# chao1224/GeoSSL

Measured on AMD Instinct MI355X. Metric: molecules/s/GPU SchNet+DDM fwd+bwd (QM9-sized, bs=1024); % HBM roofline, higher is better.
Workload: dtype f32

## Files before the change

### geossl_amd/NCSN.py

```python
import ctypes as C
import os

import numpy as np
import torch
from .switches import env as _env
import torch.nn as nn
import torch.nn.functional as F

from . import _lib
from ._lib import call, ptr, stream
from .layout import get_super_edge_layout


class MultiLayerPerceptron(nn.Module):

    def __init__(self, input_dim, hidden_dims, activation="relu", dropout=0):
        super().__init__()
        self.dims = [input_dim] + hidden_dims
        self.activation = getattr(F, activation) if isinstance(activation, str) else None
        self.dropout = nn.Dropout(dropout) if dropout else None
        self.layers = nn.ModuleList()
        for i in range(len(self.dims) - 1):
            self.layers.append(nn.Linear(self.dims[i], self.dims[i + 1]))
        self.reset_parameters()

    def reset_parameters(self):
        for layer in self.layers:
            nn.init.xavier_uniform_(layer.weight)
            nn.init.constant_(layer.bias, 0.0)

    def forward(self, input):
        from .higher_order import _linear_wide
        _lib.require_cuda(input)
        lead = input.shape[:-1]
        x = input.reshape(-1, input.shape[-1])
        for i, layer in enumerate(self.layers):
            x = _linear_wide(x, layer.weight, layer.bias)
            if i < len(self.layers) - 1:
                if self.activation:
                    x = self.activation(x)
                if self.dropout:
                    x = self.dropout(x)
        return x.reshape(*lead, x.shape[-1])


def _head_params(m):
    i, o = m.input_distance_mlp.layers, m.output_mlp.layers
    return [i[0].weight, i[0].bias, i[1].weight, i[1].bias, o[0].weight, o[0].bias, o[1].weight, o[1].bias,
            o[2].weight, o[2].bias]


_FIELDS = ("in_w1", "in_b1", "in_w2", "in_b2", "o1_w", "o1_b", "o2_w", "o2_b", "o3_w", "o3_b")

_SIDE = {"stream": None, "pending": []}


def set_side_stream(stream):
    _SIDE["stream"] = stream


def join_side_stream():
    if _SIDE["pending"]:
        for ev, _keep in _SIDE["pending"]:
            torch.cuda.current_stream().wait_event(ev)
        _SIDE["pending"].clear()


class _NcsnLoss(torch.autograd.Function):
    @staticmethod
    def forward(ctx, h, distance, noise_level, distance_noise, sel, sigmas, anneal_power, out_scale, *params):
        dev = h.device
        S, Fd = sel.S, h.size(1)
        training = ctx.needs_input_grad[0] or any(ctx.needs_input_grad[8:])
        ps = [p.detach().contiguous() for p in params]
        w = _lib.NcsnWeights()
        for name, p in zip(_FIELDS, ps):
            setattr(w, name, ptr(p))
        w.sigmas = ptr(sigmas)
        ctx.grad_slot = getattr(h, "_geossl_grad_slot", None)
        h = h.detach().contiguous()
        loss_e = torch.empty(S, dtype=torch.float32, device=dev)
        sv = None
        saved = {}
        if training:
            saved = dict(a1=torch.empty(S, Fd, dtype=torch.float32, device=dev),
                         a2=torch.empty(S, Fd // 2, dtype=torch.float32, device=dev),
                         pd=torch.empty(S, dtype=torch.float32, device=dev),
                         emb=torch.empty(S, dtype=torch.float32, device=dev),
                         gscale=torch.empty(S, dtype=torch.float32, device=dev))
            sv = _lib.NcsnSaved(*[ptr(saved[k]) for k in ("a1", "a2", "pd", "emb", "gscale")])
        lib = _lib.load()
        nws = max(int(lib.geossl_ddm_loss_fwd_workspace_floats(Fd)), 256)
        ws = (torch.empty if S > 0 else torch.zeros)(nws, dtype=torch.float32, device=dev)
        st = stream()
        call("geossl_ddm_loss_fwd", ptr(h), ptr(sel.batch), ptr(sel.sei0), ptr(sel.sei1), S,
             ptr(distance.contiguous()), ptr(noise_level.contiguous()), ptr(distance_noise.contiguous()), C.byref(w),
             Fd, float(anneal_power), ptr(loss_e), C.byref(sv) if sv is not None else None, ptr(ws), st)
        loss = torch.empty((), dtype=torch.float32, device=dev)
        call("geossl_loss_reduce_partials", ptr(ws), ptr(sel.stats), float(out_scale), ptr(loss), 0, st)
        if training:
            ctx.sel, ctx.ps, ctx.w, ctx.saved, ctx.h = sel, ps, w, saved, h
            ctx.params = params
            ctx.sigmas = sigmas
            ctx.out_scale = float(out_scale)
        return loss

    @staticmethod
    def backward(ctx, gout):
        sel, ps, w, saved, h = ctx.sel, ctx.ps, ctx.w, ctx.saved, ctx.h
        dev = h.device
        S, Fd, N = sel.S, h.size(1), h.size(0)
        st = stream()
        sv = _lib.NcsnSaved(*[ptr(saved[k]) for k in ("a1", "a2", "pd", "emb", "gscale")])
        dfeat = torch.empty(S, Fd, dtype=torch.float32, device=dev)
        demb = torch.empty(S, dtype=torch.float32, device=dev)
        grow = torch.empty(S, dtype=torch.float32, device=dev)
        gout = gout.contiguous().to(torch.float32)
        direct = _lib.direct_grads_enabled(ctx.params)
        grads = [p.grad for p in ctx.params] if direct else [torch.empty_like(p) for p in ps]
        g = _lib.NcsnGrads(*[ptr(t) for t in grads])
        lib = _lib.load()
        acc = 1 if direct else 0
        split = (_env("GEOSSL_NCSN_SPLIT_BWD") is not None or _env("GEOSSL_ARITH_24BIT") is not None
                 or max(S, N) * Fd * 4 >= 2 ** 32)
        if not split:
            ws1 = torch.empty(int(lib.geossl_ddm_loss_bwd_fused_workspace_floats(S, Fd)), dtype=torch.float32, device=dev)
            call("geossl_ddm_loss_bwd_fused", ptr(h), ptr(sel.sei0), ptr(sel.sei1), S, N, Fd, C.byref(w), C.byref(sv),
                 ptr(sel.stats), ctx.out_scale, ptr(gout), ptr(dfeat), ptr(demb), ptr(grow), C.byref(g), ptr(ws1), acc, st)
            dz1 = None
        else:
            dz1 = torch.empty(S, Fd, dtype=torch.float32, device=dev)
            call("geossl_ddm_loss_bwd_rows", C.byref(w), C.byref(sv), S, Fd, ptr(sel.stats), ctx.out_scale, ptr(gout),
                 ptr(dz1), ptr(dfeat), ptr(demb), ptr(grow), st)
        dh = None
        if ctx.needs_input_grad[0]:
            slot = ctx.grad_slot
            dh = slot.rows(N, Fd, torch.float32, dev) if slot is not None else None
            if dh is None:
                dh = torch.empty(N, Fd, dtype=torch.float32, device=dev)
            call("geossl_incidence_gather", ptr(dfeat), ptr(sel.inc_ptr), ptr(sel.inc_idx), N, Fd, ptr(dh), 0, st)
        if split:
            nfl = lib.geossl_ddm_loss_bwd_workspace_floats(S, Fd)
            side = _SIDE["stream"] if direct else None
            if side is None:
                ws = torch.empty(nfl, dtype=torch.float32, device=dev)
                call("geossl_ddm_loss_bwd_weights", ptr(h), ptr(sel.sei0), ptr(sel.sei1), S, Fd, C.byref(w), C.byref(sv),
                     ptr(dz1), ptr(demb), ptr(grow), C.byref(g), ptr(ws), acc, st)
            else:
                main = torch.cuda.current_stream()
                fork = torch.cuda.Event()
                fork.record(main)
                side.wait_event(fork)
                with torch.cuda.stream(side):
                    ws = torch.empty(nfl, dtype=torch.float32, device=dev)
                    call("geossl_ddm_loss_bwd_weights", ptr(h), ptr(sel.sei0), ptr(sel.sei1), S, Fd, C.byref(w),
                         C.byref(sv), ptr(dz1), ptr(demb), ptr(grow), C.byref(g), ptr(ws), 1, stream())
                    done = torch.cuda.Event()
                    done.record(side)
                _SIDE["pending"].append((done, (h, saved, dz1, demb, grow, ws, w, sv, ps, grads)))
        if direct:
            return (dh, None, None, None, None, None, None, None) + (None,) * len(grads)
        return (dh, None, None, None, None, None, None, None) + tuple(grads)


class _NcsnLossPair(torch.autograd.Function):

    @staticmethod
    def forward(ctx, h1, h2, d1, d2, nl1, dn1, nl2, dn2, sel, sigmas, powers, out_scale, npar, *params):
        dev = h1.device
        S, Fd, N = sel.S, h1.size(1), h1.size(0)
        training = ctx.needs_input_grad[0] or ctx.needs_input_grad[1] or any(ctx.needs_input_grad[13:])
        ps = [p.detach().contiguous() for p in params]
        pss = (ps[:npar], ps[npar:])
        dyn = getattr(sel, "dyn", None)
        ctx.dyn = dyn
        if dyn is not None:
            hs = (h1.detach().contiguous(),) * 2
            ctx.grad_slots = (None, None)
        else:
            hs = (h1.detach().contiguous(), h2.detach().contiguous())
            ctx.grad_slots = (getattr(h1, "_geossl_grad_slot", None), getattr(h2, "_geossl_grad_slot", None))
        heads = (_lib.NcsnHeadFwd * 2)()
        keep, saved, ws = [], [], []
        for k, (h, d, nl, dn) in enumerate(((hs[0], d1, nl1, dn1), (hs[1], d2, nl2, dn2))):
            hd = heads[k]
            d, nl, dn = d.contiguous(), nl.contiguous(), dn.contiguous()
            keep += [d, nl, dn]
            for name, p in zip(_FIELDS, pss[k]):
                setattr(hd.w, name, ptr(p))
            hd.w.sigmas = ptr(sigmas[k])
            hd.h, hd.distance, hd.noise_level, hd.distance_noise = ptr(h), ptr(d), ptr(nl), ptr(dn)
            hd.anneal_power = float(powers[k])
            loss_e = torch.empty(S, dtype=torch.float32, device=dev)
            sv = {}
            if training:
                sv = dict(a1=torch.empty(S, Fd, dtype=torch.float32, device=dev),
                          a2=torch.empty(S, Fd // 2, dtype=torch.float32, device=dev),
                          pd=torch.empty(S, dtype=torch.float32, device=dev),
                          emb=torch.empty(S, dtype=torch.float32, device=dev),
                          gscale=torch.empty(S, dtype=torch.float32, device=dev))
                for name in ("a1", "a2", "pd", "emb", "gscale"):
                    setattr(hd.saved, name, ptr(sv[name]))
            w_ = torch.empty(256, dtype=torch.float32, device=dev)
            hd.loss_e, hd.workspace = ptr(loss_e), ptr(w_)
            keep.append(loss_e)
            saved.append(sv)
            ws.append(w_)
        st = stream()
        call("geossl_ddm_loss_fwd2_dyn", C.byref(heads), ptr(sel.batch), ptr(sel.sei0), ptr(sel.sei1), S, Fd,
             None if dyn is None else dyn.n_super, None if dyn is None else dyn.n_atoms, st)
        loss = torch.empty((), dtype=torch.float32, device=dev)
        call("geossl_loss_reduce_partials2", ptr(ws[0]), ptr(ws[1]), ptr(sel.stats), float(out_scale), float(out_scale),
             ptr(loss), st)
        if training:
            ctx.sel, ctx.pss, ctx.saved, ctx.hs, ctx.sigmas = sel, pss, saved, hs, sigmas
            ctx.params, ctx.npar, ctx.out_scale = params, npar, float(out_scale)
        return loss

    @staticmethod
    def backward(ctx, gout):
        sel, pss, saved, hs = ctx.sel, ctx.pss, ctx.saved, ctx.hs
        dev = hs[0].device
        S, Fd, N = sel.S, hs[0].size(1), hs[0].size(0)
        st = stream()
        gout = gout.contiguous().to(torch.float32)
        direct = _lib.direct_grads_enabled(ctx.params)
        grads = [p.grad for p in ctx.params] if direct else [torch.empty_like(p) for p in pss[0] + pss[1]]
        gs = (grads[:ctx.npar], grads[ctx.npar:])
        lib = _lib.load()
        heads = (_lib.NcsnHeadBwd * 2)()
        keep, dhs = [], []
        nws = int(lib.geossl_ddm_loss_bwd_fused_workspace_floats(S, Fd))
        dyn = ctx.dyn
        dh_all = torch.empty(N, Fd, dtype=torch.float32, device=dev) if dyn is not None else None
        for k in range(2):
            hd = heads[k]
            for name, p in zip(_FIELDS, pss[k]):
                setattr(hd.w, name, ptr(p))
            hd.w.sigmas = ptr(ctx.sigmas[k])
            for name in ("a1", "a2", "pd", "emb", "gscale"):
                setattr(hd.saved, name, ptr(saved[k][name]))
            for name, t_ in zip(_FIELDS, gs[k]):
                setattr(hd.grads, name, ptr(t_))
            dfeat = torch.empty(S, Fd, dtype=torch.float32, device=dev)
            demb = torch.empty(S, dtype=torch.float32, device=dev)
            grow = torch.empty(S, dtype=torch.float32, device=dev)
            ws1 = torch.empty(nws, dtype=torch.float32, device=dev)
            slot = ctx.grad_slots[k]
            dh = dh_all if dyn is not None else (slot.rows(N, Fd, torch.float32, dev) if slot is not None else None)
            if dh is None:
                dh = torch.empty(N, Fd, dtype=torch.float32, device=dev)
            hd.h, hd.out_scale, hd.dfeat, hd.demb, hd.grow, hd.workspace, hd.dh = (
                ptr(hs[k]), ctx.out_scale, ptr(dfeat), ptr(demb), ptr(grow), ptr(ws1), ptr(dh))
            keep += [dfeat, demb, grow, ws1]
            dhs.append(dh)
        call("geossl_ddm_loss_bwd_fused2_dyn", C.byref(heads), ptr(sel.sei0), ptr(sel.sei1), S, sel.N if dyn is not None else N,
             Fd, ptr(sel.stats), ptr(gout), ptr(sel.inc_ptr), ptr(sel.inc_idx), 1 if direct else 0,
             None if dyn is None else dyn.n_super, None if dyn is None else dyn.n_atoms, st)
        head = ((dh_all, None) if dyn is not None else (dhs[0], dhs[1])) + (None,) * 11
        if direct:
            return head + (None,) * len(grads)
        return head + tuple(grads)


def ddm_heads_loss(n1, n2, data, h1, distance_1, h2, distance_2, noise_level_1=None, distance_noise_1=None,
                   noise_level_2=None, distance_noise_2=None, out_scale=0.5):
    ok = (isinstance(n1, NCSN_version_03) and isinstance(n2, NCSN_version_03) and n1.emb_dim == n2.emb_dim
          and n1.emb_dim in (32, 64, 128) and not _env("GEOSSL_NCSN_SPLIT_BWD")
          and not _env("GEOSSL_ARITH_24BIT")
          and not _env("GEOSSL_NCSN_SEPARATE_HEADS")
          and (h2 is None or h1.shape == h2.shape) and not distance_1.requires_grad and not distance_2.requires_grad
          and n1 is not n2 and not ({id(p) for p in _head_params(n1)} & {id(p) for p in _head_params(n2)}))
    if ok:
        S_, N_, Fd = data.super_edge_index.size(1), h1.size(0), h1.size(1)
        ok = S_ > 0 and max(S_, N_) * Fd * 4 < 2 ** 32
    bucket = getattr(data, "_bucket", None)
    if bucket is not None and (not ok or h2 is not None):
        raise _lib.GeosslHipError("a capacity-bucket batch needs the paired NCSN heads on one fused feature tensor")
    if not ok:
        return (n1(data, h1, distance_1, noise_level=noise_level_1, distance_noise=distance_noise_1, out_scale=out_scale) +
                n2(data, h2, distance_2, noise_level=noise_level_2, distance_noise=distance_noise_2, out_scale=out_scale))
    _lib.require_cuda(h1, h2, distance_1, distance_2, n1.sigmas, n2.sigmas)
    n1.device = n2.device = n1.sigmas.device
    num_graphs = data.num_graphs
    sel = bucket.sel if bucket is not None else get_super_edge_layout(data.batch, data.super_edge_index, num_graphs)
    draws = []
    for n_, nl, dn, d in ((n1, noise_level_1, distance_noise_1, distance_1), (n2, noise_level_2, distance_noise_2, distance_2)):
        if nl is None:
            nl = torch.randint(0, n_.sigmas.size(0), (num_graphs,), device=n_.sigmas.device)
        if dn is None:
            dn = torch.randn_like(d)
        draws.append((nl, dn))
    p1, p2 = _head_params(n1), _head_params(n2)
    return _NcsnLossPair.apply(h1, h2, distance_1.view(-1), distance_2.view(-1), draws[0][0], draws[0][1].view(-1),
                               draws[1][0], draws[1][1].view(-1), sel, (n1.sigmas.detach(), n2.sigmas.detach()),
                               (n1.anneal_power, n2.anneal_power), out_scale, len(p1), *p1, *p2)


class NCSN_version_03(torch.nn.Module):
    def __init__(self, emb_dim, sigma_begin, sigma_end, num_noise_level, noise_type, anneal_power):
        super().__init__()
        self.anneal_power = anneal_power
        self.noise_type = noise_type
        self.input_distance_mlp = MultiLayerPerceptron(1, [emb_dim, 1], activation="relu")
        self.output_mlp = MultiLayerPerceptron(1 + emb_dim, [emb_dim, emb_dim // 2, 1])
        sigmas = torch.tensor(np.exp(np.linspace(np.log(sigma_begin), np.log(sigma_end), num_noise_level)),
                              dtype=torch.float32)
        self.sigmas = nn.Parameter(sigmas, requires_grad=False)
        self.emb_dim = emb_dim

    def forward(self, data, node_feature, distance, debug=False, noise_level=None, distance_noise=None,
                out_scale=1.0):
        self.device = self.sigmas.device
        _lib.require_cuda(node_feature, distance, self.sigmas)
        if self.emb_dim not in (32, 64, 128):
            raise NotImplementedError("HIP path supports emb_dim in (32, 64, 128)")
        if distance.requires_grad:
            raise NotImplementedError("gradient w.r.t. distance/positions is not built (SURVEY.md §8(f) N3)")
        num_graphs = data.num_graphs
        sel = get_super_edge_layout(data.batch, data.super_edge_index, num_graphs)
        if noise_level is None:
            noise_level = torch.randint(0, self.sigmas.size(0), (num_graphs,), device=self.device)
        if distance_noise is None:
            distance_noise = torch.randn_like(distance)
        if sel.S == 0:
            raise ValueError("batch has no super edges (scatter_add over an empty index fails in the reference too)")
        loss = _NcsnLoss.apply(node_feature, distance.view(-1), noise_level, distance_noise.view(-1), sel,
                               self.sigmas.detach(), self.anneal_power, out_scale, *_head_params(self))
        if debug:
            print("loss", float(loss))
        return loss
```

### geossl_amd/_lib.py

```python
import ctypes as C
import os

import torch

HERE = os.path.dirname(os.path.abspath(__file__))
LIB_PATH = os.path.join(HERE, "lib", "libgeossl_hip.so")

MAX_L = 12
TN_MAX = 32
EPI_BIAS, EPI_SSP, EPI_RESIDUAL, EPI_MUL_DSSP, CHAIN_SAME_INPUT, CHAIN_NEW_INPUT, CHAIN_ADD_PREV = 1, 2, 4, 8, 16, 32, 64
EPI_SILU, EPI_MUL_DSILU = 128, 256

vp = C.c_void_p
i64 = C.c_int64
i32 = C.c_int
f32 = C.c_float
f64 = C.c_double
u64 = C.c_uint64


class FilterWeights(C.Structure):
    _fields_ = [("w1", vp * MAX_L), ("b1", vp * MAX_L), ("w2", vp * MAX_L), ("b2", vp * MAX_L)]


PREPARE_MAX = 64


class PrepareBatch(C.Structure):
    _fields_ = [("W", vp * PREPARE_MAX), ("image", vp * PREPARE_MAX), ("ldw", i32 * PREPARE_MAX), ("tb", i32 * PREPARE_MAX)]


CHAIN_MAX = 5


class ChainStage(C.Structure):
    _fields_ = [("image", vp), ("bias", vp), ("res", vp), ("tprev", vp), ("out", vp), ("ld", i32), ("flags", i32),
                ("xin", vp), ("ldxin", i32), ("pad_", i32), ("out_act", vp)]


class Chain(C.Structure):
    _fields_ = [("nstage", i32), ("st", ChainStage * CHAIN_MAX)]


LOOP_MAX_OPS = 14


class LoopOp(C.Structure):
    _fields_ = [("kind", i32), ("swap", i32), ("X", vp), ("Wf", vp), ("out", vp), ("chain", Chain)]


class FilterGradIn(C.Structure):
    _fields_ = [("x", vp * MAX_L), ("dagg", vp * MAX_L)]


class FilterGradOut(C.Structure):
    _fields_ = [("dw1", vp * MAX_L), ("db1", vp * MAX_L), ("dw2", vp * MAX_L), ("db2", vp * MAX_L)]


class TnBatch(C.Structure):
    _fields_ = [("A", vp * TN_MAX), ("B", vp * TN_MAX), ("dW", vp * TN_MAX), ("db", vp * TN_MAX)]


class NcsnWeights(C.Structure):
    _fields_ = [(k, vp) for k in ("in_w1", "in_b1", "in_w2", "in_b2", "o1_w", "o1_b", "o2_w", "o2_b", "o3_w", "o3_b",
                                  "sigmas")]


class NcsnGrads(C.Structure):
    _fields_ = [(k, vp) for k in ("in_w1", "in_b1", "in_w2", "in_b2", "o1_w", "o1_b", "o2_w", "o2_b", "o3_w", "o3_b")]


class NcsnSaved(C.Structure):
    _fields_ = [(k, vp) for k in ("a1", "a2", "pd", "emb", "gscale")]


class NcsnHeadFwd(C.Structure):
    _fields_ = [("h", vp), ("distance", vp), ("noise_level", vp), ("distance_noise", vp), ("w", NcsnWeights),
                ("saved", NcsnSaved), ("anneal_power", f32), ("pad_", f32), ("loss_e", vp), ("workspace", vp)]


class NcsnHeadBwd(C.Structure):
    _fields_ = [("h", vp), ("w", NcsnWeights), ("saved", NcsnSaved), ("out_scale", f32), ("pad_", f32), ("dfeat", vp),
                ("demb", vp), ("grow", vp), ("grads", NcsnGrads), ("workspace", vp), ("dh", vp)]


COPY_MAX = 8


class CopyBatch(C.Structure):
    _fields_ = [("dst", vp * COPY_MAX), ("src", vp * COPY_MAX), ("bytes", i64 * COPY_MAX)]


class Gather(C.Structure):
    _fields_ = [(k, vp) for k in ("x_src", "pos_src", "src_off", "mol_ptr", "x_dst", "pos_dst", "batch_dst", "se_ptr", "sei0",
                                  "sei1", "pair_ptr2", "pair_i", "pair_j", "inc_ptr", "inc_idx", "e0_src", "e1_src",
                                  "e_src_off", "e_ptr", "e0_dst", "e1_dst", "zero")] + \
               [("zero_count", i64), ("x_cols", i32), ("option", i32)]


class Mask(C.Structure):
    _fields_ = [(k, vp) for k in ("bond_ptr", "bond_dst", "src_n", "mol_id", "keep_in", "keep_out", "e_src_cnt",
                                  "e_count")] + [("seed", u64), ("max_n", i32), ("pad_", i32)]


P = C.POINTER
PROTOTYPES = {
    "geossl_abi_version": (i32, []),
    "geossl_layout_build": (i32, [vp, i64, i64, vp, vp, vp, vp]),
    "geossl_pair_index_fill": (i32, [vp, vp, i64, vp, vp, vp]),
    "geossl_radius_graph_count": (i32, [vp, vp, i64, i32, f32, i32, vp, vp]),
    "geossl_radius_graph_fill": (i32, [vp, vp, i64, i32, f32, i32, vp, vp, vp, vp, vp]),
    "geossl_pair_geometry": (i32, [vp, vp, vp, i64, i32, f32, i32, f32, vp, vp, vp, vp]),
    "geossl_rbf_fwd": (i32, [vp, i64, vp, i32, f32, vp, vp]),
    "geossl_ssp_fwd": (i32, [vp, i64, vp, vp]),
    "geossl_ssp_bwd": (i32, [vp, vp, i64, vp, vp]),
    "geossl_cfconv_filter_fwd": (i32, [vp, vp, i64, P(FilterWeights), i32, i32, i32, vp, f32, vp, vp, vp]),
    "geossl_cfconv_filter_bwd_workspace_floats": (i64, [i64, i32, i32, i32]),
    "geossl_cfconv_filter_bwd": (i32, [vp, vp, vp, vp, vp, i64, i64, P(FilterWeights), P(FilterGradIn), i32, i32, i32, vp,
                                       f32, vp, P(FilterGradOut), vp, i32, vp]),
    "geossl_cfconv_filter_dpos": (i32, [vp, vp, vp, vp, vp, i64, P(FilterWeights), P(FilterGradIn), i32, i32, i32, vp, f32,
                                        f32, vp, vp, vp, vp]),
    "geossl_pair_position_grad": (i32, [vp, vp, vp, vp, vp, i64, i64, i32, vp, vp]),
    "geossl_cfconv_aggregate": (i32, [vp, vp, vp, vp, vp, vp, i64, i32, i32, i32, vp, vp]),
    "geossl_aggregate_parts": (i32, [i32]),
    "geossl_cfconv_aggregate_work": (i32, [vp, vp, vp, vp, vp, vp, i64, i32, i32, i32, vp, vp]),
    "geossl_pair_product": (i32, [vp, vp, vp, vp, vp, i64, i32, i32, vp, vp]),
    "geossl_linear": (i32, [vp, i32, vp, vp, vp, vp, vp, i32, i64, i32, i32, i32, i32, vp]),
    "geossl_tn_plan": (None, [i64, i32, P(i32), P(i32)]),
    "geossl_tn_workspace_floats": (i64, [i64, i32, i32, i32]),
    "geossl_row_normalize_fwd": (i32, [vp, i64, i32, f32, vp, vp, vp]),
    "geossl_row_normalize_bwd": (i32, [vp, vp, vp, i64, i32, f32, vp, vp]),
    "geossl_atom_tuples": (i32, [vp, vp, i64, i32, vp, vp, vp]),
    "geossl_linear_image_words": (i64, [i32, i32]),
    "geossl_linear_prepare": (i32, [P(PrepareBatch), i32, i32, i32, i32, vp]),
    "geossl_linear_prepared": (i32, [vp, i32, vp, vp, vp, vp, vp, i32, i64, i32, i32, i32, vp]),
    "geossl_chain_image_words": (i64, [i32]),
    "geossl_chain_prepare": (i32, [P(PrepareBatch), i32, i32, i32, vp]),
    "geossl_linear_chain": (i32, [vp, i32, P(Chain), i64, i32, vp]),
    "geossl_linear_wgrad": (i32, [P(TnBatch), i32, i64, i32, i32, i32, i32, i32, vp, i32, vp]),
    "geossl_embedding_fwd": (i32, [vp, i64, vp, i32, i64, i32, vp, vp, vp]),
    "geossl_embedding_bwd_workspace_floats": (i64, [i32, i32]),
    "geossl_embedding_bwd": (i32, [vp, i64, vp, i32, i64, i32, vp, vp, i32, vp]),
    "geossl_segment_reduce_fwd": (i32, [vp, vp, i64, i32, i32, vp, vp]),
    "geossl_segment_reduce_bwd": (i32, [vp, vp, i64, i32, i32, vp, i32, vp]),
    "geossl_axpy": (i32, [vp, vp, f32, i64, vp, vp]),
    "geossl_pair_distance": (i32, [vp, vp, vp, i64, vp, vp]),
    "geossl_super_edge_ptr": (i32, [vp, vp, vp, i64, i64, vp, vp, vp]),
    "geossl_incidence_count": (i32, [vp, vp, vp, vp, i64, i32, vp, vp]),
    "geossl_incidence_fill": (i32, [vp, vp, vp, vp, i64, i32, vp, vp, vp]),
    "geossl_ddm_loss_fwd_workspace_floats": (i64, [i32]),
    "geossl_ddm_loss_fwd": (i32, [vp, vp, vp, vp, i64, vp, vp, vp, P(NcsnWeights), i32, f32, vp, P(NcsnSaved), vp, vp]),
    "geossl_schnet_layer_loop": (i32, [vp, i32, vp, i32, vp, vp, vp, i32, i32, i64, i32, i32, vp]),
    "geossl_schnet_layer_loop_ragged": (i32, [vp, i32, vp, vp, vp, i64, i32, i64, i32, vp]),
    "geossl_copy2": (i32, [vp, vp, i64, vp, vp, i64, vp]),
    "geossl_ddm_noise": (i32, [vp, f32, f32, i64, i64, i64, i32, i32, vp, vp, vp, vp, vp, vp]),
    "geossl_ddm_noise_seeded": (i32, [u64, f32, f32, i64, i64, i64, i32, i32, vp, vp, vp, vp, vp, vp]),
    "geossl_ddm_views": (i32, [vp, vp, vp, vp, i64, i64, vp, vp, vp, vp, i64, vp, vp]),
    "geossl_loss_reduce_partials": (i32, [vp, vp, f32, vp, i32, vp]),
    "geossl_ddm_loss_fwd2": (i32, [vp, vp, vp, vp, i64, i32, vp]),
    "geossl_loss_reduce_partials2": (i32, [vp, vp, vp, f32, f32, vp, vp]),
    "geossl_ddm_loss_bwd_fused2": (i32, [vp, vp, vp, i64, i64, i32, vp, vp, vp, vp, i32, vp]),
    "geossl_loss_reduce_workspace_floats": (i64, [i64]),
    "geossl_loss_reduce": (i32, [vp, i64, vp, f32, vp, vp, i32, vp]),
    "geossl_ddm_loss_bwd_rows": (i32, [P(NcsnWeights), P(NcsnSaved), i64, i32, vp, f32, vp, vp, vp, vp, vp, vp]),
    "geossl_ddm_loss_bwd_workspace_floats": (i64, [i64, i32]),
    "geossl_ddm_loss_bwd_weights": (i32, [vp, vp, vp, i64, i32, P(NcsnWeights), P(NcsnSaved), vp, vp, vp, P(NcsnGrads),
                                          vp, i32, vp]),
    "geossl_ddm_loss_bwd_fused_workspace_floats": (i64, [i64, i32]),
    "geossl_ddm_loss_bwd_fused": (i32, [vp, vp, vp, i64, i64, i32, P(NcsnWeights), P(NcsnSaved), vp, f32, vp, vp, vp, vp,
                                        P(NcsnGrads), vp, i32, vp]),
    "geossl_incidence_gather": (i32, [vp, vp, vp, i64, i32, vp, i32, vp]),
    "geossl_painn_edge_geom": (i32, [vp, vp, vp, i64, f32, vp, vp, i32, vp, vp, vp, vp]),
    "geossl_silu_fwd": (i32, [vp, i64, vp, vp]),
    "geossl_silu_bwd": (i32, [vp, vp, i64, vp, vp]),
    "geossl_painn_interaction_fwd": (i32, [vp, vp, vp, vp, vp, vp, vp, vp, vp, vp, vp, i64, i32, i32, vp, vp, vp]),
    "geossl_painn_interaction_bwd_workspace_floats": (i64, [i64, i32, i32]),
    "geossl_painn_interaction_fwd_mol": (i32, [vp, vp, vp, vp, vp, vp, vp, vp, vp, vp, vp, vp, i64, i32, i64, i32, i32, vp,
                                               vp, vp]),
    "geossl_painn_interaction_fwd_mma": (i32, [vp, vp, vp, vp, vp, vp, vp, vp, vp, vp, vp, vp, vp, i64, i32, i64, i32, i32,
                                               vp, vp, vp]),
    "geossl_painn_interaction_bwd_mol_workspace_floats": (i64, [i64, i64, i32, i32]),
    "geossl_painn_interaction_bwd_mol": (i32, [vp, vp, vp, vp, vp, vp, vp, vp, vp, vp, vp, vp, vp, i64, i32, i64, i32, i32,
                                               vp, vp, vp, vp, vp, i32, vp]),
    "geossl_painn_interaction_bwd": (i32, [vp, vp, vp, vp, vp, vp, vp, vp, vp, vp, vp, vp, i64, i32, i32, vp, vp, vp, vp,
                                           vp, i32, vp]),
    "geossl_painn_mix_pre_fwd": (i32, [vp, vp, i64, i32, f32, vp, vp, vp]),
    "geossl_painn_mix_post_fwd": (i32, [vp, vp, vp, vp, vp, i64, i32, vp, vp, vp]),
    "geossl_painn_mix_post_bwd": (i32, [vp, vp, vp, vp, vp, i64, i32, vp, vp, vp]),
    "geossl_painn_mix_pre_bwd": (i32, [vp, vp, vp, vp, i64, i32, vp, vp, vp]),
    "geossl_add": (i32, [vp, vp, i64, vp, vp]),
    "geossl_painn_edge_grads": (i32, [vp] * 11 + [i64, i32, i32, vp, vp, vp, i32, vp]),
    "geossl_painn_edge_geom_bwd": (i32, [vp, vp, vp, i64, f32, vp, vp, i32, vp, vp, vp, vp, vp]),
    "geossl_painn_position_grad": (i32, [vp, vp, vp, vp, vp, i64, vp, vp]),
    "geossl_adam_step": (i32, [vp, vp, vp, vp, i64, f64, f64, f64, f64, f64, i64, f32, vp]),
    "geossl_copy_n": (i32, [P(CopyBatch), i32, vp]),
    "geossl_ddm_views_dyn": (i32, [vp, vp, vp, vp, i64, i64, vp, vp, vp, vp, i64, vp, vp, vp, vp]),
    "geossl_embedding_fwd_dyn": (i32, [vp, i64, vp, i32, i64, i32, vp, vp, vp, vp]),
    "geossl_embedding_bwd_dyn": (i32, [vp, i64, vp, i32, i64, i32, vp, vp, i32, vp, vp]),
    "geossl_cfconv_filter_fwd_dyn": (i32, [vp, vp, i64, P(FilterWeights), i32, i32, i32, vp, f32, vp, vp, vp, vp]),
    "geossl_cfconv_filter_bwd_dyn": (i32, [vp, vp, vp, vp, vp, i64, i64, P(FilterWeights), P(FilterGradIn), i32, i32, i32,
                                           vp, f32, vp, P(FilterGradOut), vp, i32, vp, vp, vp]),
    "geossl_rbf_fragments_bytes": (i64, [i64]),
    "geossl_rbf_fragments": (i32, [vp, i64, i32, vp, f32, vp, vp]),
    "geossl_rbf_fragments_dyn": (i32, [vp, i64, i32, vp, f32, vp, vp, vp]),
    "geossl_rbf_fragment_items": (i32, [vp, i64, i32, vp, f32, vp, vp, vp]),
    "geossl_cfconv_filter_bwd_frag": (i32, [vp, vp, vp, vp, vp, i64, i64, P(FilterWeights), P(FilterGradIn), i32, i32,
                                            i32, vp, f32, vp, P(FilterGradOut), vp, i32, vp, vp]),
    "geossl_cfconv_filter_bwd_frag_dyn": (i32, [vp, vp, vp, vp, vp, i64, i64, P(FilterWeights), P(FilterGradIn), i32,
                                                i32, i32, vp, f32, vp, P(FilterGradOut), vp, i32, vp, vp, vp, vp]),
    "geossl_cfconv_aggregate_work_dyn": (i32, [vp, vp, vp, vp, vp, vp, i64, i32, i32, i32, vp, vp, vp]),
    "geossl_cfconv_aggregate_targets_dyn": (i32, [vp, vp, vp, vp, vp, vp, i64, i32, i32, i32, vp, vp, vp]),
    "geossl_linear_chain_dyn": (i32, [vp, i32, P(Chain), i64, i32, vp, vp]),
    "geossl_linear_wgrad_dyn": (i32, [P(TnBatch), i32, i64, i32, i32, i32, i32, i32, vp, i32, vp, vp]),
    "geossl_ddm_loss_fwd2_dyn": (i32, [vp, vp, vp, vp, i64, i32, vp, vp, vp]),
    "geossl_ddm_loss_bwd_fused2_dyn": (i32, [vp, vp, vp, i64, i64, i32, vp, vp, vp, vp, i32, vp, vp, vp]),
    "geossl_painn_group_capacity": (i64, [i64, i64]),
    "geossl_painn_edge_layout": (i32, [vp, vp, i64, vp, i64, i64, i64] + [vp] * 12),
    "geossl_painn_edge_layout_dyn": (i32, [vp, vp, i64, vp, vp, i64, i64, i64] + [vp] * 12),
    "geossl_painn_edge_geom_dyn": (i32, [vp, vp, vp, i64, f32, vp, vp, i32, vp, vp, vp, vp, vp]),
    "geossl_painn_interaction_fwd_mma_dyn": (i32, [vp, vp, vp, vp, vp, vp, vp, vp, vp, vp, vp, vp, vp, i64, i32, i64, i32,
                                                   i32, vp, vp, vp, vp]),
    "geossl_tape_unary": (i32, [i32, vp, i64, f32, f32, vp, vp]),
    "geossl_tape_binary": (i32, [i32, vp, i32, vp, i32, i64, i32, f32, vp, vp]),
    "geossl_tape_colsum_workspace_floats": (i64, [i64, i32]),
    "geossl_tape_reduce": (i32, [i32, vp, i64, i32, vp, vp, vp]),
    "geossl_tape_gather_rows": (i32, [vp, vp, i32, i64, i32, vp, vp]),
    "geossl_tape_scatter_rows": (i32, [vp, vp, i32, vp, i64, i32, vp, vp]),
    "geossl_tape_copy2d": (i32, [vp, i64, vp, i64, i64, i32, vp]),
    "geossl_tape_fill": (i32, [vp, i64, f32, vp]),
    "geossl_painn_stage_cap": (i32, [i32, i32, i32]),
    "geossl_painn_interaction_fwd_atoms": (i32, [vp] * 12 + [i64, vp, i32, i32, vp, vp, vp]),
    "geossl_painn_interaction_bwd_atoms": (i32, [vp] * 13 + [i64, vp, i32, i32, vp, vp, vp, vp, vp, i32, vp]),
    "geossl_painn_tile_ok": (i32, [i32, i32]),
    "geossl_painn_interaction_fwd_tile": (i32, [vp] * 12 + [i64, vp, i32, i32, vp, vp, vp]),
    "geossl_painn_interaction_bwd_tile_workspace_floats": (i64, [i64, i32, i32]),
    "geossl_painn_interaction_bwd_tile": (i32, [vp] * 13 + [i64, vp, i32, i32, vp, vp, vp, vp, vp, i32, vp]),
    "geossl_painn_interaction_bwd_mol_skip": (i32, [vp, vp, vp, vp, vp, vp, vp, vp, vp, vp, vp, vp, vp, i64, i32, i64, i32,
                                                    i32, vp, vp, vp, vp, vp, i32, vp]),
    "geossl_painn_mix_pre_fwd_dyn": (i32, [vp, vp, i64, i32, f32, vp, vp, vp, vp]),
    "geossl_painn_mix_post_fwd_dyn": (i32, [vp, vp, vp, vp, vp, i64, i32, vp, vp, vp, vp]),
    "geossl_painn_mix_post_bwd_dyn": (i32, [vp, vp, vp, vp, vp, i64, i32, vp, vp, vp, vp]),
    "geossl_painn_mix_pre_bwd_dyn": (i32, [vp, vp, vp, vp, i64, i32, vp, vp, vp, vp]),
    "geossl_gather_molecules": (i32, [P(Gather), i64, vp]),
    "geossl_gather_masked_molecules": (i32, [P(Gather), P(Mask), i64, vp]),
    "geossl_masked_edge_offsets": (i32, [vp, i64, i64, i32, vp, vp, vp, vp]),
    "geossl_infonce_fwd": (i32, [vp, vp, i64, i32, f32, vp, vp, vp, vp, vp]),
    "geossl_infonce_bwd": (i32, [vp, vp, vp, vp, i64, i32, f32, vp, vp, vp, vp]),
    "geossl_ebm_nce_fwd": (i32, [vp, vp, i64, i32, i32, vp, vp, vp, vp, vp, vp]),
    "geossl_ebm_nce_bwd": (i32, [vp, vp, vp, i64, i32, i32, vp, vp, vp, vp]),
    "geossl_distance_head_width_ok": (i32, [i32]),
    "geossl_distance_head_fwd_workspace_floats": (i64, [i64]),
    "geossl_distance_head_bwd_workspace_floats": (i64, [i64, i32]),
    "geossl_distance_head_fwd": (i32, [vp, i64, i32, vp, vp, vp, vp, vp, i64, vp, vp, vp, vp, vp, vp]),
    "geossl_distance_head_fwd_dyn": (i32, [vp, i64, i32, vp, vp, vp, vp, vp, i64, vp, vp, vp, vp, vp, vp, vp, vp]),
    "geossl_distance_head_bwd": (i32, [vp, i64, i32, vp, vp, i64, vp, vp, vp, vp, vp, vp, vp, vp, i32, vp]),
    "geossl_distance_head_bwd_dyn": (i32, [vp, i64, i32, vp, vp, i64, vp, vp, vp, vp, vp, vp, vp, vp, i32, vp, vp, vp]),
    "geossl_charge_mask_count": (i64, [i64, f64]),
    "geossl_charge_mask": (i32, [vp, i32, i64, f64, i32, vp, vp, vp, vp, vp, vp]),
    "geossl_charge_mask_dyn": (i32, [vp, i32, i64, f64, i32, vp, vp, vp, vp, vp, vp, vp]),
    "geossl_charge_head_width_ok": (i32, [i32, i32]),
    "geossl_charge_head_fwd_workspace_floats": (i64, [i64]),
    "geossl_charge_head_bwd_workspace_floats": (i64, [i64, i32, i32]),
    "geossl_charge_head_fwd": (i32, [vp, i64, i32, vp, vp, i32, vp, vp, i64, vp, vp, vp, vp, vp, vp]),
    "geossl_charge_head_fwd_dyn": (i32, [vp, i64, i32, vp, vp, i32, vp, vp, i64, vp, vp, vp, vp, vp, vp, vp]),
    "geossl_charge_head_bwd": (i32, [vp, i64, i32, vp, i32, vp, vp, i64, vp, vp, vp, vp, vp, vp, vp, i32, vp]),
    "geossl_charge_head_bwd_dyn": (i32, [vp, i64, i32, vp, i32, vp, vp, i64, vp, vp, vp, vp, vp, vp, vp, i32, vp, vp]),
    "geossl_infograph_width_ok": (i32, [i32]),
    "geossl_infograph_fwd_workspace_floats": (i64, [i64]),
    "geossl_infograph_fwd": (i32, [vp, i64, i32, vp, vp, i64, i32, vp, vp, vp, vp, vp, vp, vp, vp]),
    "geossl_infograph_fwd_dyn": (i32, [vp, i64, i32, vp, vp, i64, i32, vp, vp, vp, vp, vp, vp, vp, vp, vp]),
    "geossl_infograph_bwd": (i32, [vp, i64, i32, vp, vp, i64, i32, vp, vp, vp, vp, vp, vp, vp, vp]),
    "geossl_infograph_bwd_dyn": (i32, [vp, i64, i32, vp, vp, i64, i32, vp, vp, vp, vp, vp, vp, vp, vp, vp]),
    "geossl_property_width_ok": (i32, [i32]),
    "geossl_property_workspace_floats": (i64, [i64]),
    "geossl_property_fwd": (i32, [vp, i64, i32, vp, i64, i32, i32, vp, vp, vp, vp, vp, i64, vp, i32, vp, vp, vp, vp, vp,
                                  vp]),
    "geossl_property_fwd_dyn": (i32, [vp, i64, i32, vp, i64, i32, i32, vp, vp, vp, vp, vp, i64, vp, i32, vp, vp, vp, vp,
                                      vp, vp, vp]),
    "geossl_property_predict": (i32, [vp, i64, i32, vp, i64, i32, i32, vp, vp, vp, vp, vp, vp, vp]),
    "geossl_property_predict_dyn": (i32, [vp, i64, i32, vp, i64, i32, i32, vp, vp, vp, vp, vp, vp, vp, vp]),
    "geossl_property_bwd": (i32, [i64, i32, vp, i64, i32, i32, vp, vp, vp, vp, vp, vp, i64, vp, i32, vp, vp, vp, vp, vp,
                                  vp, i32, vp]),
    "geossl_property_bwd_dyn": (i32, [i64, i32, vp, i64, i32, i32, vp, vp, vp, vp, vp, vp, i64, vp, i32, vp, vp, vp, vp,
                                      vp, vp, i32, vp, vp]),
    "geossl_property_targets": (i32, [vp, i64, i32, i32, vp, vp, i64, vp, vp]),
    "geossl_pair_head_width_ok": (i32, [i32]),
    "geossl_pair_head_workspace_floats": (i64, [i64]),
    "geossl_pair_head_fwd": (i32, [vp, i64, i32, vp, i64, i32, vp, vp, vp, vp, vp, vp, vp, vp]),
    "geossl_pair_head_predict": (i32, [vp, i64, i32, vp, i64, i32, vp, vp, vp, vp]),
    "geossl_pair_head_bwd": (i32, [i64, i32, vp, i64, i32, vp, vp, vp, vp, vp, vp, vp, vp, vp, i32, vp]),
    "geossl_pair_head_fwd_dyn": (i32, [vp, i64, i32, vp, i64, i32, vp, vp, vp, vp, vp, vp, vp, vp, vp]),
    "geossl_pair_head_predict_dyn": (i32, [vp, i64, i32, vp, i64, i32, vp, vp, vp, vp, vp]),
    "geossl_pair_head_bwd_dyn": (i32, [i64, i32, vp, i64, i32, vp, vp, vp, vp, vp, vp, vp, vp, vp, i32, vp, vp]),
    "geossl_torsion_head_width_ok": (i32, [i32]),
    "geossl_torsion_head_fwd_workspace_floats": (i64, [i64]),
    "geossl_torsion_head_bwd_workspace_floats": (i64, [i64, i32]),
    "geossl_torsion_head_fwd": (i32, [vp, i64, i32, vp, vp, vp, vp, vp, vp, i64, vp, vp, vp, vp, vp, vp]),
    "geossl_torsion_head_fwd_dyn": (i32, [vp, i64, i32, vp, vp, vp, vp, vp, vp, i64, vp, vp, vp, vp, vp, vp, vp, vp]),
    "geossl_torsion_head_bwd": (i32, [vp, i64, i32, vp, vp, vp, vp, i64, vp, vp, i64, vp, vp, vp, vp, vp, i32, vp]),
    "geossl_torsion_head_bwd_dyn": (i32, [vp, i64, i32, vp, vp, vp, vp, i64, vp, vp, i64, vp, vp, vp, vp, vp, i32, vp, vp,
                                          vp]),
    "geossl_triple_angles": (i32, [vp, i64, vp, vp, vp, i64, vp, vp]),
    "geossl_gather_triples": (i32, [vp, i64, vp, vp, vp, vp, i64, vp, vp, vp, vp, vp]),
    "geossl_sparse_pairs_build": (i32, [vp, vp, i64, i64, i32, f32, i32, f32, i64] + [vp] * 13),
    "geossl_cfconv_aggregate_sparse": (i32, [vp, vp, vp, vp, vp, i64, i32, i32, vp, vp]),
    "geossl_sparse_pairs_build_dyn": (i32, [vp, vp, i64, i64, i32, f32, i32, f32, i64] + [vp] * 14),
    "geossl_cfconv_aggregate_sparse_dyn": (i32, [vp, vp, vp, vp, vp, i64, i32, i32, vp, vp, vp]),
    "geossl_pair_position_grad_sparse": (i32, [vp, vp, vp, vp, vp, vp, i64, i64, i32, vp, vp]),
    "geossl_pair_geometry_live": (i32, [vp, vp, vp, i64, i32, f32, i32, f32, vp, vp, vp, vp, vp]),
    "geossl_gather_live_rows": (i32, [vp, vp, vp, i64, i32, i32, vp, vp]),
    "geossl_live_pairs_build": (i32, [vp] * 8 + [i64, i64, f32] + [vp] * 9),
    "geossl_cfconv_filter_fwd_rows": (i32, [vp, vp, i64, P(FilterWeights), i32, i32, i32, vp, f32, vp, vp, vp, vp, vp]),
}

_lib = None


class GeosslHipError(RuntimeError):
    pass


def load():
    global _lib
    if _lib is not None:
        return _lib
    path = os.environ.get("GEOSSL_HIP_LIB", LIB_PATH)
    if not os.path.exists(path):
        raise GeosslHipError(
            "libgeossl_hip.so is not built (%s). Run `python -m geossl_amd.build` (needs hipcc); "
            "there is no CPU fallback." % path)
    lib = C.CDLL(path)
    for name, (res, args) in PROTOTYPES.items():
        fn = getattr(lib, name)
        fn.restype = res
        fn.argtypes = args
    if lib.geossl_abi_version() != 1:
        raise GeosslHipError("ABI version mismatch")
    _lib = lib
    return lib


def check(rc, what):
    if rc != 0:
        raise GeosslHipError("%s failed with hipError %d" % (what, rc))


def ptr(t):
    if t is None:
        return None
    return t.data_ptr()


def stream():
    return torch._C._cuda_getCurrentRawStream(torch._C._cuda_getDevice())


def require_cuda(*tensors):
    for t in tensors:
        if t is not None and not t.is_cuda:
            raise GeosslHipError(
                "geossl_amd runs on MI355X only: got a %s tensor. The HIP path has no CPU fallback." % t.device.type)



_DIRECT = {"depth": 0}


class direct_grads:
    def __enter__(self):
        _DIRECT["depth"] += 1
        return self

    def __exit__(self, *exc):
        _DIRECT["depth"] -= 1
        return False


def direct_grads_enabled(params):
    return _DIRECT["depth"] > 0 and all(
        p.grad is not None and p.grad.is_contiguous() and p.grad.dtype == torch.float32 and p.grad.is_cuda
        for p in params)


class StatusWord:

    def __init__(self, device, message):
        self.word = torch.zeros(1, dtype=torch.int32, device=device)
        self.host = torch.zeros(1, dtype=torch.int32).pin_memory()
        self.event = None
        self.message = message

    def __deepcopy__(self, memo):
        return None

    def __reduce__(self):
        return (type(None), ())

    def poll(self):
        if self.event is None or torch.cuda.is_current_stream_capturing():
            return
        if self.event.query():
            self.event = None
            if int(self.host[0]):
                raise IndexError(self.message)

    def arm(self, every=1):
        self.calls = getattr(self, "calls", 0) + 1
        if every > 1 and self.calls % every != 1:
            return
        if self.event is None and not torch.cuda.is_current_stream_capturing():
            self.host.copy_(self.word, non_blocking=True)
            self.event = torch.cuda.Event()
            self.event.record()

    def check(self):
        if int(self.word.item()):
            raise IndexError(self.message)


def module_status(module, device, message):
    st = module.__dict__.get("_geossl_status")
    if st is None or st.word.device != device:
        st = StatusWord(device, message)
        module.__dict__["_geossl_status"] = st
    return st


TIMERS = None
CALLS = None


def call(name, *args):
    global CALLS
    lib = load()
    if CALLS is not None:
        CALLS += 1
    timers = TIMERS
    key = name[:-4] if name.endswith("_dyn") else name
    if key == "geossl_cfconv_filter_fwd_rows":
        key = "geossl_cfconv_filter_fwd"
    if timers is not None and key in timers:
        e0, e1 = torch.cuda.Event(enable_timing=True), torch.cuda.Event(enable_timing=True)
        e0.record()
        rc = getattr(lib, name)(*args)
        e1.record()
        timers[key].append((e0, e1))
    else:
        rc = getattr(lib, name)(*args)
    check(rc, name)


def fill_ptrs(arr, tensors):
    for i, t in enumerate(tensors):
        arr[i] = ptr(t)
```

### geossl_amd/csrc/ncsn_bwd.hip

```cpp
#include "common.h"
#include "geossl_hip.h"
#include "split.h"
#include "tn.h"

using namespace geossl;

namespace {

constexpr int TR = 32;

#ifdef NB_TIMING
__device__ long long nb_dbg[2 * 32 * 8];
#define NB_MARK(slot)                                                                              \
  do {                                                                                             \
    if (blockIdx.x == 5 && lane == 0 && (wave == 0 || wave == NW) && t - t_begin < 32)             \
      nb_dbg[((wave == 0 ? 0 : 1) * 32 + (t - t_begin)) * 8 + (slot)] = clock64();                 \
  } while (0)
#else
#define NB_MARK(slot) do {} while (0)
#endif

template <int NW>
struct NbLds {
  static constexpr int F = 32 * NW, H = F / 2, KHS = (H + 15) / 16, HMB = (H + 31) / 32, KS = F / 16;
  u32x4* zb;
  u32x4* dz2T;
  u32x4* fT;
  u32x4* dz1r;
  u32x4* abT;
  int4* scal;
  float* pdv;
  float* dep;
  float* wls;
  int* eg;
  int* ef;
  int* ea;
  int* ec;
  __device__ explicit NbLds(uint8_t* smem) {
    zb = reinterpret_cast<u32x4*>(smem);
    dz2T = zb + 2 * KHS * 2 * 64;
    fT = dz2T + HMB * 2 * 2 * 64;
    dz1r = fT + 2 * NW * 2 * 2 * 64;
    abT = dz1r + KS * 2 * 64;
    scal = reinterpret_cast<int4*>(abT + NW * 2 * 2 * 64);
    pdv = reinterpret_cast<float*>(scal + 3 * TR);
    dep = pdv + 3 * TR;
    wls = dep + NW * TR;
    eg = reinterpret_cast<int*>(wls + F);
    ef = eg + 4;
    ea = ef + 2 * NW;
    ec = ea + NW;
  }
  static size_t bytes() {
    return (size_t)(2 * KHS * 2 + HMB * 4 + 2 * NW * 4 + KS * 2 + NW * 4) * 1024 + 3 * TR * sizeof(int4) +
           (size_t)(3 * TR + NW * TR + F) * sizeof(float) + (size_t)(4 + 4 * NW) * sizeof(int);
  }
};

struct NcsnFusedArgs {
  const float* h;
  const int64_t* sei0;
  const int64_t* sei1;
  int S;
  GeosslNcsnWeights w;
  GeosslNcsnSaved sv;
  const int64_t* divisor;
  float out_scale;
  const float* gout;
  float* dfeat;
  float* demb;
  float* grow;
  float* pw1;
  float* pd1;
  float* pb1;
  float* pw2;
  float* pb2;
  float* psm;
};

__device__ __forceinline__ float ldg_off(const float* base, uint32_t byte_off) {
  return *reinterpret_cast<const float*>(reinterpret_cast<const char*>(base) + byte_off);
}
__device__ __forceinline__ int crow4(int r, int k4) { return (r & 3) + 8 * (r >> 2) + k4; }
__device__ __forceinline__ int opaque(int v) {
  asm volatile("" : "+v"(v));
  return v;
}
__device__ __forceinline__ u32x4 pack8(const f32x16& t, int s) {
  u32x4 w;
#pragma unroll
  for (int q = 0; q < 4; ++q) {
    const f16x2 p = {(_Float16)t[8 * s + 2 * q], (_Float16)t[8 * s + 2 * q + 1]};
    w[q] = __builtin_bit_cast(uint32_t, p);
  }
  return w;
}
__device__ __forceinline__ const u32x4& piece(const Frag2& f, int pc) { return pc == 0 ? f.h : f.l; }
__device__ __forceinline__ int scale_exponent(float m) { return max(mag_exponent(m), -40); }
__device__ __forceinline__ float pow2(int e) { return __builtin_amdgcn_ldexpf(1.0f, e); }
constexpr int E_NONE = -100000;

template <int NW, bool ROLE_A>
__device__ __forceinline__ void ncsn_bwd_body(const NcsnFusedArgs& a, const int S, const float* __restrict__ a_h) {
  using L_t = NbLds<NW>;
  constexpr int F = L_t::F, H = L_t::H, KHS = L_t::KHS, HMB = L_t::HMB, KS = L_t::KS, NT = 128 * NW;
  extern __shared__ __attribute__((aligned(16))) uint8_t smem_raw[];
  const L_t L(smem_raw);
  const int tid = threadIdx.x, lane = tid & 63, j = lane & 31, kh = lane >> 5;
  const int wave = __builtin_amdgcn_readfirstlane(tid >> 6);
  const int nb = ROLE_A ? wave : wave - NW;
  const int ntiles = (S + TR - 1) / TR;
  const int per = (ntiles + (int)gridDim.x - 1) / (int)gridDim.x;
  const int t_begin = (int)blockIdx.x * per, t_end = min(ntiles, t_begin + per);
  const float scale = a.out_scale * (a.gout != nullptr ? a.gout[0] : 1.0f) / (float)a.divisor[0];
  const uint32_t col = 32 * nb + j;

  Frag2 wreg[ROLE_A ? KHS : KS];
  f32x16 accw1[ROLE_A ? NW : 1];
  f32x16 accw2[ROLE_A ? 1 : HMB];
  int E1[ROLE_A ? NW : 1];
  int E2 = E_NONE;
  int ew = 0;
  float bsum = 0.0f, dsum = 0.0f;
  u32x4 ident[2];
  float w3r[8];
  float s_w2 = 0.0f, s_w1 = 0.0f, s_b1 = 0.0f, s_g = 0.0f, s_d = 0.0f;
  float iw1 = 0.0f, ib1 = 0.0f, iw2 = 0.0f;
  int e3;
  {
    float m3 = 0.0f;
    for (int i = lane; i < H; i += 64) m3 = fmaxf(m3, fabsf(a.w.o3_w[i]));
    e3 = scale_exponent(wave_max(m3));
  }
  if constexpr (ROLE_A) {
    iw1 = a.w.in_w1[col];
    ib1 = a.w.in_b1[col];
    iw2 = a.w.in_w2[col];
    float raw[KHS][8];
    float wm = 0.0f, csum = 0.0f;
#pragma unroll
    for (int ks = 0; ks < KHS; ++ks)
#pragma unroll
      for (int e = 0; e < 8; ++e) {
        const int m = 16 * ks + 8 * kh + e;
        const float v = m < H ? a.w.o2_w[(size_t)m * F + col] : 0.0f;
        raw[ks][e] = v;
        wm = fmaxf(wm, fabsf(v));
        csum = fmaf(fabsf(v), m < H ? fabsf(a.w.o3_w[m]) : 0.0f, csum);
      }
    ew = scale_exponent(wave_max(wm));
    const float sw = pow2(14 - ew);
#pragma unroll
    for (int ks = 0; ks < KHS; ++ks) wreg[ks] = split8h_scaled(raw[ks], sw);
    csum += __shfl_xor(csum, 32, 64);
    const int ecw = max(mag_exponent(wave_max(csum)), -80);
    if (lane == 0) L.ec[nb] = ecw;
#pragma unroll
    for (int kb = 0; kb < NW; ++kb) {
      E1[kb] = E_NONE;
#pragma unroll
      for (int r = 0; r < 16; ++r) accw1[kb][r] = 0.0f;
    }
#pragma unroll
    for (int s = 0; s < 2; ++s)
#pragma unroll
      for (int q = 0; q < 4; ++q) {
        const int k0 = 16 * s + kperm(2 * q, kh), k1 = 16 * s + kperm(2 * q + 1, kh);
        ident[s][q] = (k0 == j ? 0x3C00u : 0u) | (k1 == j ? 0x3C000000u : 0u);
      }
  } else {
    float raw[KS][8];
    float wm = 0.0f;
#pragma unroll
    for (int ks = 0; ks < KS; ++ks)
#pragma unroll
      for (int e = 0; e < 8; ++e) {
        raw[ks][e] = a.w.o1_w[(size_t)(16 * ks + kperm(e, kh)) * (F + 1) + col];
        wm = fmaxf(wm, fabsf(raw[ks][e]));
      }
    ew = scale_exponent(wave_max(wm));
    const float sw = pow2(14 - ew);
#pragma unroll
    for (int ks = 0; ks < KS; ++ks) wreg[ks] = split8h_scaled(raw[ks], sw);
#pragma unroll
    for (int e = 0; e < 8; ++e) {
      const int m = 16 * nb + 8 * kh + e;
      w3r[e] = (nb < KHS && m < H) ? a.w.o3_w[m] : 0.0f;
    }
#pragma unroll
    for (int mb = 0; mb < HMB; ++mb)
#pragma unroll
      for (int r = 0; r < 16; ++r) accw2[mb][r] = 0.0f;
#pragma unroll
    for (int q2 = 0; q2 < 2; ++q2)
#pragma unroll
      for (int q = 0; q < 4; ++q) {
        const int k0 = 16 * q2 + 8 * kh + 2 * q;
        ident[q2][q] = (k0 == j ? 0x3C00u : 0u) | (k0 + 1 == j ? 0x3C000000u : 0u);
      }
  }
  for (int i = tid; i < F; i += NT) L.wls[i] = a.w.o1_w[(size_t)i * (F + 1) + F];

  int sc_u = 0, sc_v = 0;
  float sc_g = 0.0f, sc_e = 0.0f, sc_p = 0.0f;
  int EG = -60;
  auto load_scal = [&](int tt) {
    if constexpr (ROLE_A) {
      if (wave == 0) {
        const int row = min(TR * tt + j, S - 1);
        sc_u = (int)a.sei0[row];
        sc_v = (int)a.sei1[row];
        sc_g = a.sv.gscale[row];
        sc_e = a.sv.emb[row];
        sc_p = a.sv.pd[row];
      }
    }
  };
  auto put_scal = [&](int tt) {
    if constexpr (ROLE_A) {
      if (wave == 0) {
        const int row = TR * tt + lane;
        const bool valid = lane < TR && row < S && tt < t_end;
        const float gr = valid ? pin(sc_g) * scale : 0.0f;
        EG = max(EG, mag_exponent(wave_max(fabsf(gr))));
        if (lane < TR) {
          L.scal[(tt % 3) * TR + lane] = make_int4(sc_u, sc_v, __float_as_int(gr), __float_as_int(sc_e));
          L.pdv[(tt % 3) * TR + lane] = sc_p;
          if (valid) a.grow[row] = gr;
        }
        if (lane == 0) L.eg[tt % 3] = EG;
      }
    }
  };
  float a1raw[16];
  auto request_a1 = [&](int tt, int k4) {
    if constexpr (ROLE_A) {
#pragma unroll
      for (int r = 0; r < 16; ++r)
        a1raw[r] = ldg_off(a.sv.a1, ((uint32_t)min(TR * tt + crow4(r, k4), S - 1) * (uint32_t)F + col) * 4u);
    }
  };
  f32x4 a2raw[2];
  float o3acc[8] = {0.0f, 0.0f, 0.0f, 0.0f, 0.0f, 0.0f, 0.0f, 0.0f};
  auto request_a2 = [&](int tt) {
    if constexpr (!ROLE_A) {
      if (nb < KHS) {
        const uint32_t off = ((uint32_t)min(TR * tt + j, S - 1) * (uint32_t)H + (16 * nb + 8 * kh)) * 4u;
        a2raw[0] = *reinterpret_cast<const f32x4*>(reinterpret_cast<const char*>(a.sv.a2) + off);
        a2raw[1] = *reinterpret_cast<const f32x4*>(reinterpret_cast<const char*>(a.sv.a2) + 16 + off);
      }
    }
  };
  float hu[16], hv[16];
  auto request_gather = [&](int tt, int k4) {
    if constexpr (!ROLE_A) {
      const int2* sc = reinterpret_cast<const int2*>(L.scal + (tt % 3) * TR);
#pragma unroll
      for (int r = 0; r < 16; ++r) {
        const int2 uv = sc[2 * crow4(r, k4)];
        hu[r] = ldg_off(a_h, ((uint32_t)uv.x * (uint32_t)F + col) * 4u);
        hv[r] = ldg_off(a_h, ((uint32_t)uv.y * (uint32_t)F + col) * 4u);
      }
    }
  };
  auto build_zb = [&](int tt) {
    if constexpr (!ROLE_A) {
      if (nb < KHS) {
        const float gr = __int_as_float(L.scal[(tt % 3) * TR + j].z);
        const float sz = pow2(14 - e3 - __builtin_amdgcn_readfirstlane(L.eg[tt % 3]));
        const float av[8] = {a2raw[0].x, a2raw[0].y, a2raw[0].z, a2raw[0].w, a2raw[1].x, a2raw[1].y, a2raw[1].z, a2raw[1].w};
        float v[8];
#pragma unroll
        for (int e = 0; e < 8; ++e) {
          const float a2v = pin(av[e]);
          v[e] = a2v > 0.0f ? gr * w3r[e] : 0.0f;
          o3acc[e] = fmaf(gr, a2v, o3acc[e]);
        }
        const Frag2 f = split8h_scaled(v, sz);
        u32x4* dst = L.zb + (size_t)(((tt & 1) * KHS + nb) * 2) * 64 + lane;
        dst[0] = f.h;
        dst[64] = f.l;
      }
    }
  };
  int EF = -40;
  auto build_fT = [&](int tt) {
    if constexpr (!ROLE_A) {
      float v[16];
      float m = 0.0f;
#pragma unroll
      for (int r = 0; r < 16; ++r) {
        v[r] = pin(hu[r]) + pin(hv[r]);
        m = fmaxf(m, fabsf(v[r]));
      }
      EF = max(EF, mag_exponent(wave_max(m)));
      const float sf = pow2(14 - EF);
      if (lane == 0) L.ef[(tt & 1) * NW + nb] = EF;
#pragma unroll
      for (int s = 0; s < 2; ++s) {
        float vv[8];
#pragma unroll
        for (int e = 0; e < 8; ++e) vv[e] = v[8 * s + e];
        const Frag2 f = split8h_scaled(vv, sf);
        u32x4* dst = L.fT + (size_t)((((tt & 1) * NW + nb) * 2 + s) * 2) * 64 + lane;
        dst[0] = f.h;
        dst[64] = f.l;
      }
    }
  };

  load_scal(t_begin);
  put_scal(t_begin);
  load_scal(t_begin + 1);
  put_scal(t_begin + 1);
  load_scal(t_begin + 2);
  if (t_begin < t_end) {
    request_a1(t_begin, 4 * kh);
    request_a2(t_begin);
  }
  __syncthreads();
  int eC = -80;
#pragma unroll
  for (int i = 0; i < NW; ++i) eC = max(eC, __builtin_amdgcn_readfirstlane(L.ec[i]));
  if (t_begin < t_end) {
    request_gather(t_begin, 4 * kh);
    build_zb(t_begin);
    build_fT(t_begin);
    request_a2(t_begin + 1);
    request_gather(t_begin + 1, 4 * kh);
  }
  int EA = -40;
  const float kA = pow2(e3 + ew - eC - 14);
  for (int t = t_begin; t < t_end; ++t) {
    const int buf = t & 1;
    int k4 = opaque(4 * kh);
    NB_MARK(0);
    lds_barrier();
    NB_MARK(1);
    const int EGt = __builtin_amdgcn_readfirstlane(L.eg[t % 3]);
    if constexpr (ROLE_A) {
      put_scal(t + 2);
      const float kT = pow2(EGt + eC - 14);
      f32x16 acc0, acc1;
#pragma unroll
      for (int r = 0; r < 16; ++r) acc0[r] = acc1[r] = 0.0f;
      {
        const u32x4* zs = L.zb + (size_t)(buf * KHS * 2) * 64 + lane;
        Frag2 a0, an;
        a0.h = zs[0]; a0.l = zs[64];
#pragma unroll
        for (int ks = 0; ks < KHS; ++ks) {
          if (ks + 1 < KHS) {
            const u32x4* s0 = zs + (size_t)((ks + 1) * 2) * 64;
            an.h = s0[0]; an.l = s0[64];
          }
          __builtin_amdgcn_sched_barrier(0);
          mma3x2(acc0, acc1, a0, wreg[ks]);
          __builtin_amdgcn_sched_barrier(0);
          if (ks + 1 < KHS) a0 = an;
        }
      }
      NB_MARK(5);
      float v[16];
      {
        const int4* sc = L.scal + (t % 3) * TR;
        float tb = 0.0f, td = 0.0f, am = 0.0f;
#pragma unroll
        for (int r = 0; r < 16; ++r) {
          a1raw[r] = pin(a1raw[r]);
          v[r] = a1raw[r] > 0.0f ? (acc0[r] + acc1[r]) * kA : 0.0f;
          tb += v[r];
          td = fmaf(v[r], __int_as_float(sc[crow4(r, k4)].w), td);
          am = fmaxf(am, fabsf(a1raw[r]));
        }
        bsum = fmaf(tb, kT, bsum);
        dsum = fmaf(td, kT, dsum);
        EA = max(EA, mag_exponent(wave_max(am)));
      }
      {
        const float sa = pow2(14 - EA);
        if (lane == 0) L.ea[nb] = EA;
#pragma unroll
        for (int s = 0; s < 2; ++s) {
          float vv[8];
#pragma unroll
          for (int e = 0; e < 8; ++e) vv[e] = a1raw[8 * s + e];
          const Frag2 f = split8h_scaled(vv, sa);
          u32x4* dst = L.abT + (size_t)((nb * 2 + s) * 2) * 64 + lane;
          dst[0] = f.h;
          dst[64] = f.l;
        }
      }
      Frag2 da[2];
#pragma unroll
      for (int s = 0; s < 2; ++s) {
        float vv[8];
#pragma unroll
        for (int e = 0; e < 8; ++e) vv[e] = v[8 * s + e];
        da[s] = split8h(vv);
      }
      {
        float wl[16];
#pragma unroll
        for (int r = 0; r < 16; ++r) wl[r] = L.wls[32 * nb + crow4(r, k4)];
        float de = 0.0f;
#pragma unroll
        for (int pc = 1; pc >= 0; --pc) {
          f32x16 tp;
#pragma unroll
          for (int r = 0; r < 16; ++r) tp[r] = 0.0f;
          tp = mfma_f16(piece(da[0], pc), ident[0], tp);
          tp = mfma_f16(piece(da[1], pc), ident[1], tp);
#pragma unroll
          for (int r = 0; r < 16; ++r) de = fmaf(tp[r], wl[r], de);
#pragma unroll
          for (int half = 0; half < 2; ++half)
            L.dz1r[(size_t)((2 * nb + half) * 2 + pc) * 64 + lane] = pack8(tp, half);
        }
        de += __shfl_xor(de, 32, 64);
        if (kh == 0) L.dep[j * NW + nb] = de * kT;
      }
      NB_MARK(6);
#pragma unroll
      for (int kb = 0; kb < NW; ++kb) {
        const int En = EGt + __builtin_amdgcn_readfirstlane(L.ef[buf * NW + kb]);
        if (En != E1[kb]) {
          const float f = pow2(max(E1[kb] - En, -200));
#pragma unroll
          for (int r = 0; r < 16; ++r) accw1[kb][r] *= f;
          E1[kb] = En;
        }
#pragma unroll
        for (int s = 0; s < 2; ++s) {
          const u32x4* s0 = L.fT + (size_t)(((buf * NW + kb) * 2 + s) * 2) * 64 + lane;
          Frag2 bf;
          bf.h = s0[0]; bf.l = s0[64];
          mma3(accw1[kb], da[s], bf);
        }
      }
    } else {
      if (nb < HMB) {
        float tb = 0.0f;
#pragma unroll
        for (int pc = 1; pc >= 0; --pc) {
          f32x16 tp;
#pragma unroll
          for (int r = 0; r < 16; ++r) tp[r] = 0.0f;
#pragma unroll
          for (int q = 0; q < 2; ++q) {
            if (2 * nb + q < KHS) {
              const u32x4* s0 = L.zb + (size_t)((buf * KHS + 2 * nb + q) * 2 + pc) * 64 + lane;
              tp = mfma_f16(s0[0], ident[q], tp);
            }
          }
#pragma unroll
          for (int r = 0; r < 16; ++r) tb += tp[r];
#pragma unroll
          for (int s = 0; s < 2; ++s) L.dz2T[(size_t)((nb * 2 + s) * 2 + pc) * 64 + lane] = pack8(tp, s);
        }
        bsum = fmaf(tb, pow2(EGt + e3 - 14), bsum);
      }
      NB_MARK(5);
      build_zb(t + 1);
      NB_MARK(6);
      build_fT(t + 1);
    }
    k4 = opaque(4 * kh);
    NB_MARK(2);
    lds_barrier();
    NB_MARK(3);
    if constexpr (ROLE_A) {
      request_a1(t + 1, k4);
      load_scal(t + 3);
      {
        const int4* sc = L.scal + (t % 3) * TR;
        const float* pdr = L.pdv + (t % 3) * TR;
#pragma unroll
        for (int i = 0; i < 16; ++i) {
          const int rl = 4 * k4 + i;
          float de = 0.0f;
#pragma unroll
          for (int n2 = 0; n2 < NW; ++n2) de += L.dep[rl * NW + n2];
          const float pd = pdr[rl];
          const float pre = fmaf(iw1, pd, ib1);
          s_w2 = fmaf(de, fmaxf(pre, 0.0f), s_w2);
          const float dp = pre > 0.0f ? de * iw2 : 0.0f;
          s_w1 = fmaf(dp, pd, s_w1);
          s_b1 += dp;
          if (wave == 0 && j == i) {
            s_g += __int_as_float(sc[rl].z);
            s_d += de;
          }
        }
      }
    } else {
      request_a2(t + 2);
      request_gather(t + 2, k4);
      NB_MARK(7);
      f32x16 acc0, acc1;
#pragma unroll
      for (int r = 0; r < 16; ++r) acc0[r] = acc1[r] = 0.0f;
      {
        const u32x4* zs = L.dz1r + lane;
        Frag2 b0, bn;
        b0.h = zs[0]; b0.l = zs[64];
#pragma unroll
        for (int ks = 0; ks < KS; ++ks) {
          if (ks + 1 < KS) {
            const u32x4* s0 = zs + (size_t)((ks + 1) * 2) * 64;
            bn.h = s0[0]; bn.l = s0[64];
          }
          __builtin_amdgcn_sched_barrier(0);
          mma3x2(acc0, acc1, wreg[ks], b0);
          __builtin_amdgcn_sched_barrier(0);
          if (ks + 1 < KS) b0 = bn;
        }
      }
      const float kD = pow2(EGt + eC + ew - 28);
      f32x16 outp;
#pragma unroll
      for (int r = 0; r < 16; ++r) outp[r] = (acc0[r] + acc1[r]) * kD;
      const int row = TR * t + j;
      if (row < S) {
        const uint32_t off = ((uint32_t)row * (uint32_t)F + 32 * nb + 4 * kh) * 4u;
#pragma unroll
        for (int q = 0; q < 4; ++q)
          *reinterpret_cast<f32x4*>(reinterpret_cast<char*>(a.dfeat) + 32 * q + off) =
              f32x4{outp[4 * q], outp[4 * q + 1], outp[4 * q + 2], outp[4 * q + 3]};
        if (nb == 0 && kh == 0) {
          float de = 0.0f;
#pragma unroll
          for (int n2 = 0; n2 < NW; ++n2) de += L.dep[j * NW + n2];
          a.demb[row] = de;
        }
      }
      {
        const int En = EGt + __builtin_amdgcn_readfirstlane(L.ea[nb]);
        if (En != E2) {
          const float f = pow2(max(E2 - En, -200));
#pragma unroll
          for (int mb = 0; mb < HMB; ++mb)
#pragma unroll
            for (int r = 0; r < 16; ++r) accw2[mb][r] *= f;
          E2 = En;
        }
      }
#pragma unroll
      for (int s = 0; s < 2; ++s) {
        const u32x4* sb = L.abT + (size_t)((nb * 2 + s) * 2) * 64 + lane;
        Frag2 bf;
        bf.h = sb[0]; bf.l = sb[64];
#pragma unroll
        for (int mb = 0; mb < HMB; ++mb) {
          const u32x4* s0 = L.dz2T + (size_t)((mb * 2 + s) * 2) * 64 + lane;
          Frag2 af;
          af.h = s0[0]; af.l = s0[64];
          mma3(accw2[mb], af, bf);
        }
      }
    }
    NB_MARK(4);
  }
  const size_t pb = blockIdx.x;
  if constexpr (ROLE_A) {
    float* P1 = a.pw1 + pb * F * F;
#pragma unroll
    for (int kb = 0; kb < NW; ++kb) {
      const float f = pow2(max(E1[kb] + eC - 28, -200));
#pragma unroll
      for (int r = 0; r < 16; ++r) P1[(size_t)(32 * nb + c_row(r, lane)) * F + 32 * kb + j] = accw1[kb][r] * f;
    }
    const float sb = bsum + __shfl_xor(bsum, 32, 64), sd = dsum + __shfl_xor(dsum, 32, 64);
    if (kh == 0) {
      a.pb1[pb * F + col] = sb;
      a.pd1[pb * F + col] = sd;
    }
    float* Ps = a.psm + pb * (H + 3 * F + 2);
    const float t_w2 = s_w2 + __shfl_xor(s_w2, 32, 64);
    const float t_w1 = s_w1 + __shfl_xor(s_w1, 32, 64), t_b1 = s_b1 + __shfl_xor(s_b1, 32, 64);
    if (kh == 0) {
      Ps[H + col] = t_w2;
      Ps[H + F + col] = t_w1;
      Ps[H + 2 * F + col] = t_b1;
    }
    if (wave == 0) {
      const float tg = wave_sum(s_g), td = wave_sum(s_d);
      if (lane == 0) {
        Ps[H + 3 * F] = tg;
        Ps[H + 3 * F + 1] = td;
      }
    }
  } else {
    float* P2 = a.pw2 + pb * H * F;
    const float f = pow2(max(E2 + e3 - 28, -200));
#pragma unroll
    for (int mb = 0; mb < HMB; ++mb)
#pragma unroll
      for (int r = 0; r < 16; ++r) {
        const int m = 32 * mb + c_row(r, lane);
        if (m < H) P2[(size_t)m * F + col] = accw2[mb][r] * f;
      }
    const float sb = bsum + __shfl_xor(bsum, 32, 64);
    if (nb < HMB && kh == 0 && (int)col < H) a.pb2[pb * H + col] = sb;
    if (nb < KHS) {
      float* Ps = a.psm + pb * (H + 3 * F + 2);
#pragma unroll
      for (int e = 0; e < 8; ++e) {
        float v = o3acc[e];
#pragma unroll
        for (int o = 16; o > 0; o >>= 1) v += __shfl_xor(v, o, 64);
        const int m = 16 * nb + 8 * kh + e;
        if (j == 0 && m < H) Ps[m] = v;
      }
    }
  }
}

template <int NW>
__global__ __launch_bounds__(128 * NW) void k_ncsn_bwd_fused(NcsnFusedArgs a) {
  if ((int)(threadIdx.x >> 6) < NW) ncsn_bwd_body<NW, true>(a, a.S, a.h);
  else ncsn_bwd_body<NW, false>(a, a.S, a.h);
}
struct NcsnFusedPair { NcsnFusedArgs a[2]; };
template <int NW>
__global__ __launch_bounds__(128 * NW) void k_ncsn_bwd_fused2(NcsnFusedPair pr, const int32_t* __restrict__ dyn_S,
                                                              const int32_t* __restrict__ dyn_view) {
  const NcsnFusedArgs& a = pr.a[blockIdx.y];
  const int S = dyn_count(a.S, dyn_S);
  const float* h = a.h;
  if (dyn_view != nullptr && blockIdx.y == 1) h += (size_t)(*dyn_view) * (32 * NW);
  if ((int)(threadIdx.x >> 6) < NW) ncsn_bwd_body<NW, true>(a, S, h);
  else ncsn_bwd_body<NW, false>(a, S, h);
}

__device__ __forceinline__ void ncsn_reduce_all_block(const ReduceMulti& m, int nblk, int accumulate,
                                                      const float* __restrict__ psm, int F, const GeosslNcsnGrads& g,
                                                      float (*red)[64]) {
  const int mb = m.xoff[m.nseg];
  if ((int)blockIdx.x < mb) {
    reduce_multi_block(m, nblk, accumulate, red, 0);
    return;
  }
  const int H = F / 2, len = H + 3 * F + 2;
  const int i = ((int)blockIdx.x - mb) * 4 + (int)(threadIdx.x >> 6), lane = threadIdx.x & 63;
  if (i >= len) return;
  float s = 0.0f;
  for (int b = lane; b < nblk; b += 64) s += psm[(size_t)b * len + i];
  s = wave_sum(s);
  if (lane == 0) {
    float* dst;
    if (i < H) dst = g.o3_w + i;
    else if (i < H + F) dst = g.in_w2 + (i - H);
    else if (i < H + 2 * F) dst = g.in_w1 + (i - H - F);
    else if (i < H + 3 * F) dst = g.in_b1 + (i - H - 2 * F);
    else if (i == H + 3 * F) dst = g.o3_b;
    else dst = g.in_b2;
    *dst = accumulate ? *dst + s : s;
  }
}
__global__ __launch_bounds__(256) void k_ncsn_reduce_all(ReduceMulti m, int nblk, int accumulate,
                                                         const float* __restrict__ psm, int F, GeosslNcsnGrads g) {
  __shared__ float red[4][64];
  ncsn_reduce_all_block(m, nblk, accumulate, psm, F, g, red);
}
__global__ __launch_bounds__(256) void k_ncsn_reduce_all2(ReduceMulti m0, ReduceMulti m1, int nblk, int accumulate,
                                                          const float* __restrict__ psm0,
                                                          const float* __restrict__ psm1, int F, GeosslNcsnGrads g0,
                                                          GeosslNcsnGrads g1) {
  __shared__ float red[4][64];
  if (blockIdx.y == 0) ncsn_reduce_all_block(m0, nblk, accumulate, psm0, F, g0, red);
  else ncsn_reduce_all_block(m1, nblk, accumulate, psm1, F, g1, red);
}

inline int fused_blocks(int64_t S) {
  const int64_t ntiles = (S + TR - 1) / TR;
  return (int)(ntiles < 256 ? ntiles : 256);
}

}

#ifdef NB_TIMING
extern "C" int geossl_ncsn_bwd_debug_read(long long* host) {
  return (int)hipMemcpyFromSymbol(host, HIP_SYMBOL(nb_dbg), sizeof(long long) * 2 * 32 * 8);
}
#endif

extern "C" int64_t geossl_ddm_loss_bwd_fused_workspace_floats(int64_t S, int F) {
  const int64_t nb = fused_blocks(S), H = F / 2;
  return nb * ((int64_t)F * F + 2 * F + H * F + H + (H + 3 * F + 2));
}

extern "C" int geossl_ddm_loss_bwd_fused(const float* h, const int64_t* sei0, const int64_t* sei1, int64_t S, int64_t N,
                                         int F, const GeosslNcsnWeights* w, const GeosslNcsnSaved* saved,
                                         const int64_t* stats_divisor, float out_scale, const float* gout, float* dfeat,
                                         float* demb, float* grow, const GeosslNcsnGrads* grads, float* workspace,
                                         int accumulate, hipStream_t stream) {
  if (S <= 0) return 0;
  if (F != 32 && F != 64 && F != 128) return (int)hipErrorInvalidValue;
  if (S * (int64_t)F * 4 >= ((int64_t)1 << 32) || N * (int64_t)F * 4 >= ((int64_t)1 << 32)) return (int)hipErrorInvalidValue;
  const int nb = fused_blocks(S), H = F / 2;
  NcsnFusedArgs a;
  a.h = h; a.sei0 = sei0; a.sei1 = sei1; a.S = (int)S; a.w = *w; a.sv = *saved; a.divisor = stats_divisor;
  a.out_scale = out_scale; a.gout = gout; a.dfeat = dfeat; a.demb = demb; a.grow = grow;
  a.pw1 = workspace;
  a.pd1 = a.pw1 + (size_t)nb * F * F;
  a.pb1 = a.pd1 + (size_t)nb * F;
  a.pw2 = a.pb1 + (size_t)nb * F;
  a.pb2 = a.pw2 + (size_t)nb * H * F;
  a.psm = a.pb2 + (size_t)nb * H;
#define LAUNCH(NWV)                                                                                      \
  do {                                                                                                   \
    allow_big_lds(&k_ncsn_bwd_fused<NWV>);                                                               \
    hipLaunchKernelGGL((k_ncsn_bwd_fused<NWV>), dim3(nb), dim3(128 * NWV), NbLds<NWV>::bytes(), stream, a); \
  } while (0)
  if (F == 128) LAUNCH(4); else if (F == 64) LAUNCH(2); else LAUNCH(1);
#undef LAUNCH
  GEOSSL_CHECK_LAUNCH();
  ReduceMulti rm;
  float* o1w[1] = {grads->o1_w};
  float* o1c[1] = {grads->o1_w + F};
  float* o1b[1] = {grads->o1_b};
  float* o2w[1] = {grads->o2_w};
  float* o2b[1] = {grads->o2_b};
  rm.add(a.pw1, F * F, F, F + 1, 1, o1w, 1);
  rm.add(a.pd1, F, F, F, F + 1, o1c, 1);
  rm.add(a.pb1, F, F, F, 1, o1b, 1);
  rm.add(a.pw2, H * F, F, F, 1, o2w, 1);
  rm.add(a.pb2, H, H, H, 1, o2b, 1);
  hipLaunchKernelGGL(k_ncsn_reduce_all, dim3(rm.blocks() + (H + 3 * F + 2 + 3) / 4, 1), dim3(256), 0, stream, rm, nb,
                     accumulate, a.psm, F, *grads);
  GEOSSL_CHECK_LAUNCH();
  return 0;
}

namespace geossl {
int launch_incidence_gather2(const float* dfeat0, const float* dfeat1, const int64_t* inc_ptr, const int32_t* inc_idx,
                             int64_t N, int F, float* dh0, float* dh1, hipStream_t stream, const int32_t* dyn_view);
}

extern "C" int geossl_ddm_loss_bwd_fused2(const GeosslNcsnHeadBwd* heads, const int64_t* sei0, const int64_t* sei1,
                                          int64_t S, int64_t N, int F, const int64_t* stats_divisor, const float* gout,
                                          const int64_t* inc_ptr, const int32_t* inc_idx, int accumulate,
                                          hipStream_t stream) {
  return geossl_ddm_loss_bwd_fused2_dyn(heads, sei0, sei1, S, N, F, stats_divisor, gout, inc_ptr, inc_idx, accumulate,
                                        nullptr, nullptr, stream);
}

extern "C" int geossl_ddm_loss_bwd_fused2_dyn(const GeosslNcsnHeadBwd* heads, const int64_t* sei0, const int64_t* sei1,
                                              int64_t S, int64_t N, int F, const int64_t* stats_divisor,
                                              const float* gout, const int64_t* inc_ptr, const int32_t* inc_idx,
                                              int accumulate, const int32_t* dyn_S, const int32_t* dyn_view,
                                              hipStream_t stream) {
  if (S <= 0) return 0;
  if (heads == nullptr || (F != 32 && F != 64 && F != 128)) return (int)hipErrorInvalidValue;
  if (S * (int64_t)F * 4 >= ((int64_t)1 << 32) || N * (int64_t)F * 4 >= ((int64_t)1 << 32)) return (int)hipErrorInvalidValue;
  const int nb = (fused_blocks(S) + 1) / 2, H = F / 2;
  NcsnFusedPair pr;
  NcsnFusedArgs* a = pr.a;
  for (int k = 0; k < 2; ++k) {
    const GeosslNcsnHeadBwd& hd = heads[k];
    if (hd.h == nullptr || hd.dfeat == nullptr || hd.workspace == nullptr) return (int)hipErrorInvalidValue;
    NcsnFusedArgs& x = a[k];
    x.h = hd.h; x.sei0 = sei0; x.sei1 = sei1; x.S = (int)S; x.w = hd.w; x.sv = hd.saved; x.divisor = stats_divisor;
    x.out_scale = hd.out_scale; x.gout = gout; x.dfeat = hd.dfeat; x.demb = hd.demb; x.grow = hd.grow;
    x.pw1 = hd.workspace;
    x.pd1 = x.pw1 + (size_t)nb * F * F;
    x.pb1 = x.pd1 + (size_t)nb * F;
    x.pw2 = x.pb1 + (size_t)nb * F;
    x.pb2 = x.pw2 + (size_t)nb * H * F;
    x.psm = x.pb2 + (size_t)nb * H;
  }
#define LAUNCH2(NWV)                                                                                                \
  do {                                                                                                              \
    allow_big_lds(&k_ncsn_bwd_fused2<NWV>);                                                                         \
    hipLaunchKernelGGL((k_ncsn_bwd_fused2<NWV>), dim3(nb, 2), dim3(128 * NWV), NbLds<NWV>::bytes(), stream, pr,         \
                       dyn_S, dyn_view);                                                                            \
  } while (0)
  if (F == 128) LAUNCH2(4); else if (F == 64) LAUNCH2(2); else LAUNCH2(1);
#undef LAUNCH2
  GEOSSL_CHECK_LAUNCH();
  ReduceMulti rm[2];
  for (int k = 0; k < 2; ++k) {
    const GeosslNcsnGrads* grads = &heads[k].grads;
    float* o1w[1] = {grads->o1_w};
    float* o1c[1] = {grads->o1_w + F};
    float* o1b[1] = {grads->o1_b};
    float* o2w[1] = {grads->o2_w};
    float* o2b[1] = {grads->o2_b};
    rm[k].add(a[k].pw1, F * F, F, F + 1, 1, o1w, 1);
    rm[k].add(a[k].pd1, F, F, F, F + 1, o1c, 1);
    rm[k].add(a[k].pb1, F, F, F, 1, o1b, 1);
    rm[k].add(a[k].pw2, H * F, F, F, 1, o2w, 1);
    rm[k].add(a[k].pb2, H, H, H, 1, o2b, 1);
  }
  hipLaunchKernelGGL(k_ncsn_reduce_all2, dim3(rm[0].blocks() + (H + 3 * F + 2 + 3) / 4, 2), dim3(256), 0, stream, rm[0],
                     rm[1], nb, accumulate, a[0].psm, a[1].psm, F, heads[0].grads, heads[1].grads);
  GEOSSL_CHECK_LAUNCH();
  if (heads[0].dh != nullptr && heads[1].dh != nullptr)
    return launch_incidence_gather2(heads[0].dfeat, heads[1].dfeat, inc_ptr, inc_idx, N, F, heads[0].dh, heads[1].dh, stream,
                                    dyn_view);
  return 0;
}
```

### include/geossl_hip.h

```cpp
#ifndef GEOSSL_HIP_H
#define GEOSSL_HIP_H
#include <stdint.h>
#ifdef __HIPCC__
#include <hip/hip_runtime.h>
#else
typedef struct ihipStream_t* hipStream_t;
#endif

#ifdef __cplusplus
extern "C" {
#endif

#define GEOSSL_ABI_VERSION 1
#define GEOSSL_MAX_L 12
#define GEOSSL_TN_MAX 32
#define GEOSSL_LOSS_PARTIALS 256

#define GEOSSL_EPI_BIAS 1
#define GEOSSL_EPI_SSP 2
#define GEOSSL_EPI_RESIDUAL 4
#define GEOSSL_EPI_MUL_DSSP 8
#define GEOSSL_CHAIN_NEW_INPUT 32
#define GEOSSL_CHAIN_ADD_PREV 64
#define GEOSSL_EPI_SILU 128
#define GEOSSL_EPI_MUL_DSILU 256
#define GEOSSL_CHAIN_SAME_INPUT 16

int geossl_abi_version(void);

int geossl_layout_build(const int64_t* batch, int64_t N, int64_t B, int32_t* mol_ptr, int32_t* pair_ptr,
                        int64_t* stats, hipStream_t stream);
int geossl_atom_tuples(const int32_t* mol_ptr, const int64_t* tuple_ptr, int64_t B, int option, int64_t* out0,
                       int64_t* out1, hipStream_t stream);
int geossl_pair_index_fill(const int32_t* mol_ptr, const int32_t* pair_ptr, int64_t B, int32_t* pair_i,
                           int32_t* pair_j, hipStream_t stream);

int geossl_radius_graph_count(const float* pos, const int32_t* mol_ptr, int64_t B, int max_n, float r2, int cap,
                              int32_t* deg, hipStream_t stream);
int geossl_radius_graph_fill(const float* pos, const int32_t* mol_ptr, int64_t B, int max_n, float r2, int cap,
                             const int64_t* edge_ptr, int64_t* edge_src, int64_t* edge_dst, float* edge_weight,
                             hipStream_t stream);
int geossl_pair_geometry(const float* pos, const int32_t* mol_ptr, const int32_t* pair_ptr, int64_t B, int max_n,
                         float r2, int cap, float cutoff, float* pair_d, float* pair_c, uint8_t* pair_flag,
                         hipStream_t stream);

int geossl_rbf_fwd(const float* d, int64_t E, const float* offset, int G, float coeff, float* out,
                   hipStream_t stream);

int geossl_ssp_fwd(const float* x, int64_t n, float* y, hipStream_t stream);
int geossl_ssp_bwd(const float* y, const float* dy, int64_t n, float* dx, hipStream_t stream);

typedef struct {
  const float* w1[GEOSSL_MAX_L];
  const float* b1[GEOSSL_MAX_L];
  const float* w2[GEOSSL_MAX_L];
  const float* b2[GEOSSL_MAX_L];
} GeosslFilterWeights;
int geossl_cfconv_filter_fwd(const float* pair_d, const float* pair_c, int64_t P, const GeosslFilterWeights* w, int L,
                             int F, int G, const float* offset, float coeff, float* T, float* Wf, hipStream_t stream);

typedef struct {
  const float* x[GEOSSL_MAX_L];
  const float* dagg[GEOSSL_MAX_L];
} GeosslFilterGradIn;
typedef struct {
  float* dw1[GEOSSL_MAX_L];
  float* db1[GEOSSL_MAX_L];
  float* dw2[GEOSSL_MAX_L];
  float* db2[GEOSSL_MAX_L];
} GeosslFilterGradOut;
int64_t geossl_cfconv_filter_bwd_workspace_floats(int64_t P, int L, int F, int G);
int geossl_cfconv_filter_bwd(const float* pair_d, const float* pair_c, const uint8_t* pair_flag, const int32_t* pair_i,
                             const int32_t* pair_j, int64_t P, int64_t N, const GeosslFilterWeights* w,
                             const GeosslFilterGradIn* g, int L, int F, int G, const float* offset, float coeff,
                             const float* T, const GeosslFilterGradOut* out, float* workspace, int accumulate,
                             hipStream_t stream);

int geossl_cfconv_filter_dpos(const float* pair_d, const float* pair_c, const uint8_t* pair_flag, const int32_t* pair_i,
                              const int32_t* pair_j, int64_t P, const GeosslFilterWeights* w,
                              const GeosslFilterGradIn* g, int L, int F, int G, const float* offset, float coeff,
                              float cutoff, const float* T, const float* Wf, float* dd, hipStream_t stream);
int geossl_pair_position_grad(const float* pos, const float* pair_d, const float* dd, const int32_t* mol_ptr,
                              const int32_t* pair_ptr, int64_t B, int64_t P, int L, float* dpos, hipStream_t stream);

int geossl_cfconv_aggregate(const float* x, const float* Wf, const uint8_t* pair_flag, const int32_t* mol_ptr,
                            const int32_t* pair_ptr, const int32_t* order, int64_t B, int max_n, int F, int swap,
                            float* out, hipStream_t stream);
int geossl_aggregate_parts(int n);
int geossl_cfconv_aggregate_targets_dyn(const float* x, const float* Wf, const uint8_t* pair_flag, const int32_t* mol_ptr,
                                        const int32_t* pair_ptr, const int32_t* work, int64_t nwork, int max_n, int F,
                                        int swap, float* out, const int32_t* dyn_nwork, hipStream_t stream);
int geossl_cfconv_aggregate_work(const float* x, const float* Wf, const uint8_t* pair_flag, const int32_t* mol_ptr,
                                 const int32_t* pair_ptr, const int32_t* work, int64_t nwork, int max_n, int F,
                                 int swap, float* out, hipStream_t stream);

int geossl_pair_product(const float* a, const float* b, const int32_t* pair_i, const int32_t* pair_j,
                        const uint8_t* pair_flag, int64_t P, int F, int swap, float* out, hipStream_t stream);

int geossl_linear(const float* X, int ldx, const float* W, const float* bias, const float* res, const float* tprev,
                  float* Y, int ldy, int64_t R, int K, int NO, int transB, int flags, hipStream_t stream);

#define GEOSSL_PREPARE_MAX 64
typedef struct {
  const float* W[GEOSSL_PREPARE_MAX];
  uint32_t* image[GEOSSL_PREPARE_MAX];
  int ldw[GEOSSL_PREPARE_MAX];
  int tb[GEOSSL_PREPARE_MAX];
} GeosslPrepareBatch;
int64_t geossl_linear_image_words(int K, int NO);
int geossl_linear_prepare(const GeosslPrepareBatch* batch, int nprob, int K, int NO, int transB, hipStream_t stream);
int geossl_linear_prepared(const float* X, int ldx, const uint32_t* image, const float* bias, const float* res,
                           const float* tprev, float* Y, int ldy, int64_t R, int K, int NO, int flags,
                           hipStream_t stream);

#define GEOSSL_CHAIN_MAX 5
typedef struct {
  const uint32_t* image;
  const float* bias;
  const float* res;
  const float* tprev;
  float* out;
  int ld;
  int flags;
  const float* xin;
  int ldxin;
  int pad_;
  float* out_act;
} GeosslChainStage;
typedef struct {
  int nstage;
  GeosslChainStage st[GEOSSL_CHAIN_MAX];
} GeosslChain;
int64_t geossl_chain_image_words(int F);
int geossl_chain_prepare(const GeosslPrepareBatch* batch, int nprob, int F, int transB, hipStream_t stream);
int geossl_linear_chain(const float* X, int ldx, const GeosslChain* chain, int64_t R, int F, hipStream_t stream);

#define GEOSSL_LOOP_MAX_OPS 14
typedef struct {
  int kind;
  int swap;
  const float* X;
  const float* Wf;
  float* out;
  GeosslChain chain;
} GeosslLoopOp;
int geossl_schnet_layer_loop(const GeosslLoopOp* ops, int nops, const int32_t* plan, int nblocks, const int32_t* mol_ptr,
                             const int32_t* pair_ptr, const uint8_t* pair_flag, int max_n, int uniform, int64_t N, int F,
                             int stagger, hipStream_t stream);
int geossl_schnet_layer_loop_ragged(const GeosslLoopOp* ops, int nops, const int32_t* mol_ptr, const int32_t* pair_ptr,
                                    const uint8_t* pair_flag, int64_t B, int mols_per_block, int64_t N, int F,
                                    hipStream_t stream);

typedef struct {
  const float* A[GEOSSL_TN_MAX];
  const float* B[GEOSSL_TN_MAX];
  float* dW[GEOSSL_TN_MAX];
  float* db[GEOSSL_TN_MAX];
} GeosslTnBatch;
typedef struct {
  float* out[GEOSSL_TN_MAX];
} GeosslReduceBatch;
void geossl_tn_plan(int64_t R, int nprob, int* chunk, int* nblk);
int64_t geossl_tn_workspace_floats(int64_t R, int M, int N, int nprob);
int geossl_linear_wgrad(const GeosslTnBatch* batch, int nprob, int64_t R, int M, int N, int lda, int ldb, int ldw,
                        float* workspace, int accumulate, hipStream_t stream);

int geossl_embedding_fwd(const int64_t* z, int64_t z_stride, const float* table, int num_classes, int64_t N, int F,
                         float* out, int32_t* status, hipStream_t stream);
int64_t geossl_embedding_bwd_workspace_floats(int num_classes, int F);
int geossl_embedding_bwd(const int64_t* z, int64_t z_stride, const float* dh, int num_classes, int64_t N, int F,
                         float* dtable, float* workspace, int accumulate, hipStream_t stream);

int geossl_segment_reduce_fwd(const float* h, const int32_t* mol_ptr, int64_t B, int F, int mean, float* out,
                              hipStream_t stream);
int geossl_row_normalize_fwd(const float* h, int64_t N, int F, float eps, float* y, float* norm, hipStream_t stream);
int geossl_row_normalize_bwd(const float* g, const float* y, const float* norm, int64_t N, int F, float eps,
                             float* dh, hipStream_t stream);
int geossl_segment_reduce_bwd(const float* dout, const int32_t* mol_ptr, int64_t B, int F, int mean, float* dh,
                              int accumulate, hipStream_t stream);

int geossl_axpy(const float* a, const float* b, float alpha, int64_t n, float* out, hipStream_t stream);
int geossl_pair_distance(const float* pos, const int64_t* sei0, const int64_t* sei1, int64_t S, float* out,
                         hipStream_t stream);
int geossl_copy2(void* dst0, const void* src0, int64_t bytes0, void* dst1, const void* src1, int64_t bytes1,
                 hipStream_t stream);
int geossl_ddm_noise(const int64_t* seed, float mu, float sigma, int64_t n_pos, int64_t S, int64_t B, int K1, int K2,
                     float* pos_noise, int64_t* noise_level_1, float* distance_noise_1, int64_t* noise_level_2,
                     float* distance_noise_2, hipStream_t stream);
int geossl_ddm_noise_seeded(uint64_t seed, float mu, float sigma, int64_t n_pos, int64_t S, int64_t B, int K1, int K2,
                            float* pos_noise, int64_t* noise_level_1, float* distance_noise_1, int64_t* noise_level_2,
                            float* distance_noise_2, hipStream_t stream);
int geossl_ddm_views(const float* pos, const float* noise, const int64_t* sei0, const int64_t* sei1, int64_t N, int64_t S,
                     float* pos2, float* d01, float* d02, const int64_t* z, int64_t z_stride, int64_t* z2,
                     hipStream_t stream);
int geossl_super_edge_ptr(const int64_t* batch, const int64_t* sei0, const int64_t* sei1, int64_t S, int64_t B,
                          int32_t* se_ptr, int64_t* stats, hipStream_t stream);
int geossl_incidence_count(const int64_t* batch, const int64_t* sei0, const int64_t* sei1, const int32_t* se_ptr,
                           int64_t N, int sides, int32_t* inc_cnt, hipStream_t stream);
int geossl_incidence_fill(const int64_t* batch, const int64_t* sei0, const int64_t* sei1, const int32_t* se_ptr,
                          int64_t N, int sides, const int64_t* inc_ptr, int32_t* inc_idx, hipStream_t stream);

typedef struct {
  const float* in_w1;
  const float* in_b1;
  const float* in_w2;
  const float* in_b2;
  const float* o1_w;
  const float* o1_b;
  const float* o2_w;
  const float* o2_b;
  const float* o3_w;
  const float* o3_b;
  const float* sigmas;
} GeosslNcsnWeights;
typedef struct {
  float* in_w1; float* in_b1; float* in_w2; float* in_b2;
  float* o1_w; float* o1_b; float* o2_w; float* o2_b; float* o3_w; float* o3_b;
} GeosslNcsnGrads;
typedef struct {
  float* a1; float* a2; float* pd; float* emb; float* gscale;
} GeosslNcsnSaved;
int64_t geossl_ddm_loss_fwd_workspace_floats(int F);
int geossl_ddm_loss_fwd(const float* h, const int64_t* batch, const int64_t* sei0, const int64_t* sei1, int64_t S,
                        const float* distance, const int64_t* noise_level, const float* distance_noise,
                        const GeosslNcsnWeights* w, int F, float anneal_power, float* loss_e,
                        const GeosslNcsnSaved* saved, float* workspace, hipStream_t stream);
int64_t geossl_loss_reduce_workspace_floats(int64_t S);
int geossl_loss_reduce(const float* loss_e, int64_t S, const int64_t* stats_divisor, float out_scale, float* loss,
                       float* workspace, int accumulate, hipStream_t stream);
typedef struct {
  const float* h;
  const float* distance;
  const int64_t* noise_level;
  const float* distance_noise;
  GeosslNcsnWeights w;
  GeosslNcsnSaved saved;
  float anneal_power;
  float pad_;
  float* loss_e;
  float* workspace;
} GeosslNcsnHeadFwd;
typedef struct {
  const float* h;
  GeosslNcsnWeights w;
  GeosslNcsnSaved saved;
  float out_scale;
  float pad_;
  float* dfeat;
  float* demb;
  float* grow;
  GeosslNcsnGrads grads;
  float* workspace;
  float* dh;
} GeosslNcsnHeadBwd;
int geossl_ddm_loss_fwd2(const GeosslNcsnHeadFwd* heads, const int64_t* batch, const int64_t* sei0, const int64_t* sei1,
                         int64_t S, int F, hipStream_t stream);
int geossl_loss_reduce_partials2(const float* partial0, const float* partial1, const int64_t* stats_divisor, float scale0,
                                 float scale1, float* loss, hipStream_t stream);
int geossl_ddm_loss_bwd_fused2(const GeosslNcsnHeadBwd* heads, const int64_t* sei0, const int64_t* sei1, int64_t S,
                               int64_t N, int F, const int64_t* stats_divisor, const float* gout, const int64_t* inc_ptr,
                               const int32_t* inc_idx, int accumulate, hipStream_t stream);
int geossl_loss_reduce_partials(const float* partial, const int64_t* stats_divisor, float out_scale, float* loss,
                                int accumulate, hipStream_t stream);
int geossl_ddm_loss_bwd_rows(const GeosslNcsnWeights* w, const GeosslNcsnSaved* saved, int64_t S, int F,
                             const int64_t* stats_divisor, float out_scale, const float* gout, float* dz1,
                             float* dfeat, float* demb, float* grow, hipStream_t stream);
int64_t geossl_ddm_loss_bwd_workspace_floats(int64_t S, int F);
int geossl_ddm_loss_bwd_weights(const float* h, const int64_t* sei0, const int64_t* sei1, int64_t S, int F,
                                const GeosslNcsnWeights* w, const GeosslNcsnSaved* saved, const float* dz1,
                                const float* demb, const float* grow, const GeosslNcsnGrads* grads,
                                float* workspace, int accumulate, hipStream_t stream);
int64_t geossl_ddm_loss_bwd_fused_workspace_floats(int64_t S, int F);
int geossl_ddm_loss_bwd_fused(const float* h, const int64_t* sei0, const int64_t* sei1, int64_t S, int64_t N, int F,
                              const GeosslNcsnWeights* w, const GeosslNcsnSaved* saved, const int64_t* stats_divisor,
                              float out_scale, const float* gout, float* dfeat, float* demb, float* grow,
                              const GeosslNcsnGrads* grads, float* workspace, int accumulate, hipStream_t stream);
int geossl_incidence_gather(const float* dfeat, const int64_t* inc_ptr, const int32_t* inc_idx, int64_t N, int F,
                            float* dh, int accumulate, hipStream_t stream);

int geossl_painn_edge_geom(const float* pos, const int64_t* idx_i, const int64_t* idx_j, int64_t E, float cutoff,
                           const float* offsets, const float* widths, int R, float* dir, float* fcut, float* phi,
                           hipStream_t stream);
int geossl_silu_fwd(const float* u, int64_t n, float* y, hipStream_t stream);
int geossl_silu_bwd(const float* u, const float* dy, int64_t n, float* du, hipStream_t stream);
int geossl_painn_interaction_fwd(const float* q, const float* mu, const float* xc, const int64_t* idx_j,
                                 const int64_t* inc_ptr, const int32_t* inc_idx, const float* phi, const float* fcut,
                                 const float* dir, const float* Wf, const float* bf, int64_t N, int F, int R,
                                 float* q_out, float* mu_out, hipStream_t stream);
int64_t geossl_painn_interaction_bwd_workspace_floats(int64_t N, int F, int R);
int geossl_painn_interaction_bwd(const float* dq_out, const float* dmu_out, const float* mu, const float* xc,
                                 const int64_t* idx_i, const int64_t* inc_ptr, const int32_t* inc_idx, const float* phi,
                                 const float* fcut, const float* dir, const float* Wf, const float* bf, int64_t N, int F,
                                 int R, float* dxc, float* dmu_in, float* dWf, float* dbf, float* workspace,
                                 int accumulate, hipStream_t stream);
int geossl_painn_interaction_fwd_mma(const float* q, const float* mu, const float* xc, const int64_t* idx_j,
                                     const int32_t* row_edge, const int32_t* grp_atom, const int32_t* mol_grp,
                                     const float* phi, const float* fcut, const float* dir, const float* Wf,
                                     const float* bf, const int32_t* mol_ptr, int64_t B, int max_n, int64_t N, int F, int R,
                                     float* q_out, float* mu_out, hipStream_t stream);
int geossl_painn_interaction_fwd_mol(const float* q, const float* mu, const float* xc, const int64_t* idx_j,
                                     const int64_t* inc_ptr, const int32_t* inc_idx, const float* phi, const float* fcut,
                                     const float* dir, const float* Wf, const float* bf, const int32_t* mol_ptr,
                                     int64_t B, int max_n, int64_t N, int F, int R, float* q_out, float* mu_out,
                                     hipStream_t stream);
int64_t geossl_painn_interaction_bwd_mol_workspace_floats(int64_t N, int64_t B, int F, int R);
int geossl_painn_interaction_bwd_mol(const float* dq_out, const float* dmu_out, const float* mu, const float* xc,
                                     const int64_t* idx_i, const int64_t* inc_ptr, const int32_t* inc_idx,
                                     const float* phi, const float* fcut, const float* dir, const float* Wf,
                                     const float* bf, const int32_t* mol_ptr, int64_t B, int max_n, int64_t N, int F,
                                     int R, float* dxc, float* dmu_in, float* dWf, float* dbf, float* workspace,
                                     int accumulate, hipStream_t stream);
int geossl_painn_mix_pre_fwd(const float* q, const float* mm, int64_t N, int F, float eps, float* ctx, float* dot,
                             hipStream_t stream);
int geossl_painn_mix_post_fwd(const float* q, const float* mu, const float* mm, const float* xx, const float* dot,
                              int64_t N, int F, float* q_out, float* mu_out, hipStream_t stream);
int geossl_painn_mix_post_bwd(const float* dq_new, const float* dmu_new, const float* mm, const float* xx,
                              const float* dot, int64_t N, int F, float* dxx, float* dmm, hipStream_t stream);
int geossl_painn_mix_pre_bwd(const float* dq_new, const float* dctx, const float* ctx, const float* mm, int64_t N, int F,
                             float* dq_in, float* dmm, hipStream_t stream);
int geossl_add(const float* a, const float* b, int64_t n, float* out, hipStream_t stream);

int geossl_painn_edge_grads(const float* dq_out, const float* dmu_out, const float* mu, const float* xc,
                            const int64_t* idx_i, const int64_t* idx_j, const float* phi, const float* fcut,
                            const float* dir, const float* Wf, const float* bf, int64_t E, int F, int R, float* dphi,
                            float* dfcut, float* ddir, int accumulate, hipStream_t stream);
int geossl_painn_edge_geom_bwd(const float* pos, const int64_t* idx_i, const int64_t* idx_j, int64_t E, float cutoff,
                               const float* offsets, const float* widths, int R, const float* dphi, const float* dfcut,
                               const float* ddir, float* dr, hipStream_t stream);
int geossl_painn_position_grad(const float* dr, const int64_t* inc_i_ptr, const int32_t* inc_i_idx,
                               const int64_t* inc_j_ptr, const int32_t* inc_j_idx, int64_t N, float* dpos,
                               hipStream_t stream);

int geossl_adam_step(float* param, const float* grad, float* exp_avg, float* exp_avg_sq, int64_t n, double lr,
                     double beta1, double beta2, double eps, double weight_decay, int64_t step_count, float grad_scale,
                     hipStream_t stream);

#define GEOSSL_COPY_MAX 8
typedef struct GeosslCopyBatch {
  void* dst[GEOSSL_COPY_MAX];
  const void* src[GEOSSL_COPY_MAX];
  int64_t bytes[GEOSSL_COPY_MAX];
} GeosslCopyBatch;
int geossl_copy_n(const GeosslCopyBatch* batch, int n, hipStream_t stream);
int geossl_ddm_views_dyn(const float* pos, const float* noise, const int64_t* sei0, const int64_t* sei1, int64_t N,
                         int64_t S, float* pos2, float* d01, float* d02, const int64_t* z, int64_t z_stride, int64_t* z2,
                         const int32_t* dyn_N, const int32_t* dyn_S, hipStream_t stream);
int geossl_embedding_fwd_dyn(const int64_t* z, int64_t z_stride, const float* table, int num_classes, int64_t N, int F,
                             float* out, int32_t* status, const int32_t* dyn_N, hipStream_t stream);
int geossl_embedding_bwd_dyn(const int64_t* z, int64_t z_stride, const float* dh, int num_classes, int64_t N, int F,
                             float* dtable, float* workspace, int accumulate, const int32_t* dyn_N, hipStream_t stream);
int geossl_cfconv_filter_fwd_dyn(const float* pair_d, const float* pair_c, int64_t P, const GeosslFilterWeights* w, int L,
                                 int F, int G, const float* offset, float coeff, float* T, float* Wf,
                                 const int32_t* dyn_P, hipStream_t stream);
int geossl_cfconv_filter_bwd_dyn(const float* pair_d, const float* pair_c, const uint8_t* pair_flag,
                                 const int32_t* pair_i, const int32_t* pair_j, int64_t P, int64_t N,
                                 const GeosslFilterWeights* w, const GeosslFilterGradIn* g, int L, int F, int G,
                                 const float* offset, float coeff, const float* T, const GeosslFilterGradOut* out,
                                 float* workspace, int accumulate, const int32_t* dyn_P, const int32_t* dyn_N,
                                 hipStream_t stream);
int64_t geossl_rbf_fragments_bytes(int64_t P);
int geossl_rbf_fragments(const float* pair_d, int64_t P, int G, const float* offset, float coeff, void* image,
                         hipStream_t stream);
int geossl_rbf_fragments_dyn(const float* pair_d, int64_t P, int G, const float* offset, float coeff, void* image,
                             const int32_t* dyn_P, hipStream_t stream);
int geossl_rbf_fragment_items(const float* pair_d, int64_t P, int G, const float* offset, float coeff, void* items,
                              const int32_t* dyn_P, hipStream_t stream);
int geossl_cfconv_filter_bwd_frag(const float* pair_d, const float* pair_c, const uint8_t* pair_flag,
                                  const int32_t* pair_i, const int32_t* pair_j, int64_t P, int64_t N,
                                  const GeosslFilterWeights* w, const GeosslFilterGradIn* g, int L, int F, int G,
                                  const float* offset, float coeff, const float* T, const GeosslFilterGradOut* out,
                                  float* workspace, int accumulate, const void* image, hipStream_t stream);
int geossl_cfconv_filter_bwd_frag_dyn(const float* pair_d, const float* pair_c, const uint8_t* pair_flag,
                                      const int32_t* pair_i, const int32_t* pair_j, int64_t P, int64_t N,
                                      const GeosslFilterWeights* w, const GeosslFilterGradIn* g, int L, int F, int G,
                                      const float* offset, float coeff, const float* T, const GeosslFilterGradOut* out,
                                      float* workspace, int accumulate, const int32_t* dyn_P, const int32_t* dyn_N,
                                      const void* image, hipStream_t stream);
int geossl_cfconv_aggregate_work_dyn(const float* x, const float* Wf, const uint8_t* pair_flag, const int32_t* mol_ptr,
                                     const int32_t* pair_ptr, const int32_t* work, int64_t nwork, int max_n, int F,
                                     int swap, float* out, const int32_t* dyn_nwork, hipStream_t stream);
int geossl_linear_chain_dyn(const float* X, int ldx, const GeosslChain* chain, int64_t R, int F, const int32_t* dyn_R,
                            hipStream_t stream);
int geossl_linear_wgrad_dyn(const GeosslTnBatch* batch, int nprob, int64_t R, int M, int N, int lda, int ldb, int ldw,
                            float* workspace, int accumulate, const int32_t* dyn_R, hipStream_t stream);
int geossl_ddm_loss_fwd2_dyn(const GeosslNcsnHeadFwd* heads, const int64_t* batch, const int64_t* sei0,
                             const int64_t* sei1, int64_t S, int F, const int32_t* dyn_S, const int32_t* dyn_view,
                             hipStream_t stream);
int geossl_ddm_loss_bwd_fused2_dyn(const GeosslNcsnHeadBwd* heads, const int64_t* sei0, const int64_t* sei1, int64_t S,
                                   int64_t N, int F, const int64_t* stats_divisor, const float* gout,
                                   const int64_t* inc_ptr, const int32_t* inc_idx, int accumulate, const int32_t* dyn_S,
                                   const int32_t* dyn_view, hipStream_t stream);

int64_t geossl_painn_group_capacity(int64_t E2, int64_t N2);
int geossl_painn_edge_layout(const int64_t* src_i, const int64_t* src_j, int64_t E, const int32_t* mol_ptr, int64_t N,
                             int64_t B, int64_t N2cap, int64_t* idx_i2, int64_t* idx_j2, int64_t* iptr_i,
                             int32_t* ilist_i, int64_t* iptr_j, int32_t* ilist_j, int32_t* row_edge, int32_t* grp_atom,
                             int32_t* mol_grp, int32_t* mol_grp_end, int32_t* status, hipStream_t stream);
int geossl_painn_edge_layout_dyn(const int64_t* src_i, const int64_t* src_j, int64_t E_cap, const int32_t* dyn_E,
                                 const int32_t* mol_ptr, int64_t N, int64_t B, int64_t N2cap, int64_t* idx_i2,
                                 int64_t* idx_j2, int64_t* iptr_i, int32_t* ilist_i, int64_t* iptr_j, int32_t* ilist_j,
                                 int32_t* row_edge, int32_t* grp_atom, int32_t* mol_grp, int32_t* mol_grp_end,
                                 int32_t* status, hipStream_t stream);
int geossl_painn_edge_geom_dyn(const float* pos, const int64_t* idx_i, const int64_t* idx_j, int64_t E, float cutoff,
                               const float* offsets, const float* widths, int R, float* dir, float* fcut, float* phi,
                               const int32_t* dyn_E, hipStream_t stream);
int geossl_painn_interaction_fwd_mma_dyn(const float* q, const float* mu, const float* xc, const int64_t* idx_j,
                                         const int32_t* row_edge, const int32_t* grp_atom, const int32_t* mol_grp,
                                         const float* phi, const float* fcut, const float* dir, const float* Wf,
                                         const float* bf, const int32_t* mol_ptr, int64_t B, int max_n, int64_t N, int F,
                                         int R, float* q_out, float* mu_out, const int32_t* mol_grp_end,
                                         hipStream_t stream);
int geossl_painn_stage_cap(int kind, int F, int R);
int geossl_painn_interaction_fwd_atoms(const float* q, const float* mu, const float* xc, const int64_t* idx_j,
                                       const int64_t* inc_ptr, const int32_t* inc_idx, const float* phi,
                                       const float* fcut, const float* dir, const float* Wf, const float* bf,
                                       const int32_t* atom_list, int64_t nlist, const int32_t* dyn_nlist, int F, int R,
                                       float* q_out, float* mu_out, hipStream_t stream);
int geossl_painn_interaction_bwd_atoms(const float* dq_out, const float* dmu_out, const float* mu, const float* xc,
                                       const int64_t* idx_i, const int64_t* inc_ptr, const int32_t* inc_idx,
                                       const float* phi, const float* fcut, const float* dir, const float* Wf,
                                       const float* bf, const int32_t* atom_list, int64_t nlist,
                                       const int32_t* dyn_nlist, int F, int R, float* dxc, float* dmu_in, float* dWf,
                                       float* dbf, float* workspace, int accumulate, hipStream_t stream);
int geossl_painn_interaction_bwd_mol_skip(const float* dq_out, const float* dmu_out, const float* mu, const float* xc,
                                          const int64_t* idx_i, const int64_t* inc_ptr, const int32_t* inc_idx,
                                          const float* phi, const float* fcut, const float* dir, const float* Wf,
                                          const float* bf, const int32_t* mol_ptr, int64_t B, int max_n, int64_t N, int F,
                                          int R, float* dxc, float* dmu_in, float* dWf, float* dbf, float* workspace,
                                          int accumulate, hipStream_t stream);
int geossl_painn_mix_pre_fwd_dyn(const float* q, const float* mm, int64_t N, int F, float eps, float* ctx, float* dot,
                                 const int32_t* dyn_N, hipStream_t stream);
int geossl_painn_mix_post_fwd_dyn(const float* q, const float* mu, const float* mm, const float* xx, const float* dot,
                                  int64_t N, int F, float* q_out, float* mu_out, const int32_t* dyn_N,
                                  hipStream_t stream);
int geossl_painn_mix_post_bwd_dyn(const float* dq_new, const float* dmu_new, const float* mm, const float* xx,
                                  const float* dot, int64_t N, int F, float* dxx, float* dmm, const int32_t* dyn_N,
                                  hipStream_t stream);
int geossl_painn_mix_pre_bwd_dyn(const float* dq_new, const float* dctx, const float* ctx, const float* mm, int64_t N,
                                 int F, float* dq_in, float* dmm, const int32_t* dyn_N, hipStream_t stream);

int geossl_painn_tile_ok(int F, int R);
int geossl_painn_interaction_fwd_tile(const float* q, const float* mu, const float* xc, const int64_t* idx_j,
                                      const int64_t* inc_ptr, const int32_t* inc_idx, const float* phi,
                                      const float* fcut, const float* dir, const float* Wf, const float* bf,
                                      const int32_t* atom_list, int64_t nlist, const int32_t* dyn_nlist, int F, int R,
                                      float* q_out, float* mu_out, hipStream_t stream);
int64_t geossl_painn_interaction_bwd_tile_workspace_floats(int64_t nlist, int F, int R);
int geossl_painn_interaction_bwd_tile(const float* dq_out, const float* dmu_out, const float* mu, const float* xc,
                                      const int64_t* idx_i, const int64_t* inc_ptr, const int32_t* inc_idx,
                                      const float* phi, const float* fcut, const float* dir, const float* Wf,
                                      const float* bf, const int32_t* atom_list, int64_t nlist,
                                      const int32_t* dyn_nlist, int F, int R, float* dxc, float* dmu_in, float* dWf,
                                      float* dbf, float* workspace, int accumulate, hipStream_t stream);

int geossl_tape_unary(int kind, const float* x, int64_t n, float alpha, float beta, float* y, hipStream_t stream);
int geossl_tape_binary(int op, const float* a, int amode, const float* b, int bmode, int64_t R, int D, float scale,
                       float* y, hipStream_t stream);
int64_t geossl_tape_colsum_workspace_floats(int64_t R, int D);
int geossl_tape_reduce(int kind, const float* x, int64_t R, int D, float* y, float* workspace, hipStream_t stream);
int geossl_tape_gather_rows(const float* src, const void* idx, int idx64, int64_t E, int D, float* out,
                            hipStream_t stream);
int geossl_tape_scatter_rows(const float* src, const void* ptr, int ptr64, const int32_t* perm, int64_t N, int D,
                             float* out, hipStream_t stream);
int geossl_tape_copy2d(const float* src, int64_t ld_src, float* dst, int64_t ld_dst, int64_t R, int C,
                       hipStream_t stream);
int geossl_tape_fill(float* dst, int64_t n, float value, hipStream_t stream);

typedef struct GeosslGather {
  const int64_t* x_src;
  const float* pos_src;
  const int32_t* src_off;
  const int32_t* mol_ptr;
  int64_t* x_dst;
  float* pos_dst;
  int64_t* batch_dst;
  const int32_t* se_ptr;
  int64_t* sei0;
  int64_t* sei1;
  const int32_t* pair_ptr2;
  int32_t* pair_i;
  int32_t* pair_j;
  const int64_t* inc_ptr;
  int32_t* inc_idx;
  const int64_t* e0_src;
  const int64_t* e1_src;
  const int32_t* e_src_off;
  const int32_t* e_ptr;
  int64_t* e0_dst;
  int64_t* e1_dst;
  float* zero;
  int64_t zero_count;
  int32_t x_cols;
  int32_t option;
} GeosslGather;
int geossl_gather_molecules(const GeosslGather* g, int64_t B, hipStream_t stream);

typedef struct GeosslMask {
  const int32_t* bond_ptr;
  const int32_t* bond_dst;
  const int32_t* src_n;
  const int64_t* mol_id;
  const int32_t* keep_in;
  int32_t* keep_out;
  const int32_t* e_src_cnt;
  int32_t* e_count;
  uint64_t seed;
  int32_t max_n;
  int32_t pad_;
} GeosslMask;
int geossl_gather_masked_molecules(const GeosslGather* g, const GeosslMask* mask, int64_t B, hipStream_t stream);

int geossl_masked_edge_offsets(const int32_t* e_count, int64_t B, int64_t E_cap, int views, int32_t* e_ptr,
                               int32_t* dyn_E2, int32_t* status, hipStream_t stream);

int geossl_infonce_fwd(const float* X, const float* Y, int64_t B, int F, float inv_t, float* stats, int32_t* amax,
                       float* loss, int32_t* counts, hipStream_t stream);
int geossl_infonce_bwd(const float* X, const float* Y, const float* stats, const int32_t* amax, int64_t B, int F,
                       float inv_t, const float* gout, float* dX, float* dY, hipStream_t stream);
int geossl_ebm_nce_fwd(const float* X, const float* Y, int64_t B, int F, int num_neg, float* pred, double* terms,
                       int32_t* hits, double* loss, int32_t* counts, hipStream_t stream);
int geossl_ebm_nce_bwd(const float* X, const float* Y, const float* pred, int64_t B, int F, int num_neg,
                       const double* gout, float* dX, float* dY, hipStream_t stream);

int geossl_distance_head_width_ok(int F);
int64_t geossl_distance_head_fwd_workspace_floats(int64_t S);
int64_t geossl_distance_head_bwd_workspace_floats(int64_t N, int F);
int geossl_distance_head_fwd(const float* h, int64_t N, int F, const float* W, const float* bias, const float* pos,
                             const int64_t* sei0, const int64_t* sei1, int64_t S, float* proj, float* pred, float* sgn,
                             float* workspace, float* loss, hipStream_t stream);
int geossl_distance_head_fwd_dyn(const float* h, int64_t N, int F, const float* W, const float* bias, const float* pos,
                                 const int64_t* sei0, const int64_t* sei1, int64_t S, float* proj, float* pred,
                                 float* sgn, float* workspace, float* loss, const int32_t* dyn_N, const int32_t* dyn_S,
                                 hipStream_t stream);
int geossl_distance_head_bwd(const float* h, int64_t N, int F, const float* W, const int64_t* sei0, int64_t S,
                             const float* sgn, const int64_t* inc_ptr, const int32_t* inc_idx, const float* gout,
                             float* dh, float* dW, float* db, float* workspace, int accumulate, hipStream_t stream);
int geossl_distance_head_bwd_dyn(const float* h, int64_t N, int F, const float* W, const int64_t* sei0, int64_t S,
                                 const float* sgn, const int64_t* inc_ptr, const int32_t* inc_idx, const float* gout,
                                 float* dh, float* dW, float* db, float* workspace, int accumulate,
                                 const int32_t* dyn_N, const int32_t* dyn_S, hipStream_t stream);

int64_t geossl_charge_mask_count(int64_t N, double ratio);
int geossl_charge_mask(int64_t* x, int x_cols, int64_t N, double ratio, int C, int64_t* seed, const int64_t* given,
                       int64_t* idx, int64_t* labels, int32_t* k, hipStream_t stream);
int geossl_charge_mask_dyn(int64_t* x, int x_cols, int64_t N, double ratio, int C, int64_t* seed, const int64_t* given,
                           int64_t* idx, int64_t* labels, int32_t* k, const int32_t* dyn_N, hipStream_t stream);
int geossl_charge_head_width_ok(int F, int C);
int64_t geossl_charge_head_fwd_workspace_floats(int64_t K);
int64_t geossl_charge_head_bwd_workspace_floats(int64_t K, int F, int C);
int geossl_charge_head_fwd(const float* h, int64_t N, int F, const float* W, const float* bias, int C,
                           const int64_t* idx, const int64_t* labels, int64_t K, const int32_t* k_dev, float* prob,
                           float* workspace, float* loss, int32_t* status, hipStream_t stream);
int geossl_charge_head_fwd_dyn(const float* h, int64_t N, int F, const float* W, const float* bias, int C,
                               const int64_t* idx, const int64_t* labels, int64_t K, const int32_t* k_dev, float* prob,
                               float* workspace, float* loss, int32_t* status, const int32_t* dyn_N,
                               hipStream_t stream);
int geossl_charge_head_bwd(const float* h, int64_t N, int F, const float* W, int C, const int64_t* idx,
                           const int64_t* labels, int64_t K, const int32_t* k_dev, const float* prob, const float* gout,
                           float* dh, float* dW, float* db, float* workspace, int accumulate, hipStream_t stream);
int geossl_charge_head_bwd_dyn(const float* h, int64_t N, int F, const float* W, int C, const int64_t* idx,
                               const int64_t* labels, int64_t K, const int32_t* k_dev, const float* prob,
                               const float* gout, float* dh, float* dW, float* db, float* workspace, int accumulate,
                               const int32_t* dyn_N, hipStream_t stream);

int geossl_infograph_width_ok(int F);
int64_t geossl_infograph_fwd_workspace_floats(int64_t B);
int geossl_infograph_fwd(const float* x, int64_t N, int F, const float* W, const int32_t* mol_ptr, int64_t B,
                         int readout, const float* m_in, float* s, float* h, float* scores, float* workspace,
                         float* loss, int32_t* counts, hipStream_t stream);
int geossl_infograph_fwd_dyn(const float* x, int64_t N, int F, const float* W, const int32_t* mol_ptr, int64_t B,
                             int readout, const float* m_in, float* s, float* h, float* scores, float* workspace,
                             float* loss, int32_t* counts, const int32_t* dyn_N, hipStream_t stream);
int geossl_infograph_bwd(const float* x, int64_t N, int F, const float* W, const int32_t* mol_ptr, int64_t B,
                         int readout, const float* s, const float* h, const float* scores, const float* gout,
                         float* dx, float* dm, float* dh, hipStream_t stream);
int geossl_infograph_bwd_dyn(const float* x, int64_t N, int F, const float* W, const int32_t* mol_ptr, int64_t B,
                             int readout, const float* s, const float* h, const float* scores, const float* gout,
                             float* dx, float* dm, float* dh, const int32_t* dyn_N, hipStream_t stream);

int geossl_property_width_ok(int F);
int64_t geossl_property_workspace_floats(int64_t B);
int geossl_property_fwd(const float* h, int64_t N, int F, const int32_t* mol_ptr, int64_t B, int readout, int head,
                        const float* W1, const float* b1, const float* W2, const float* b2, const float* y,
                        int64_t y_stride, const float* stats, int loss_kind, float* m, float* z, float* pred,
                        float* workspace, float* loss, hipStream_t stream);
int geossl_property_fwd_dyn(const float* h, int64_t N, int F, const int32_t* mol_ptr, int64_t B, int readout, int head,
                            const float* W1, const float* b1, const float* W2, const float* b2, const float* y,
                            int64_t y_stride, const float* stats, int loss_kind, float* m, float* z, float* pred,
                            float* workspace, float* loss, const int32_t* dyn_N, hipStream_t stream);
int geossl_property_predict(const float* h, int64_t N, int F, const int32_t* mol_ptr, int64_t B, int readout, int head,
                            const float* W1, const float* b1, const float* W2, const float* b2, const float* stats,
                            float* pred, hipStream_t stream);
int geossl_property_predict_dyn(const float* h, int64_t N, int F, const int32_t* mol_ptr, int64_t B, int readout,
                                int head, const float* W1, const float* b1, const float* W2, const float* b2,
                                const float* stats, float* pred, const int32_t* dyn_N, hipStream_t stream);
int geossl_property_bwd(int64_t N, int F, const int32_t* mol_ptr, int64_t B, int readout, int head, const float* W1,
                        const float* W2, const float* m, const float* z, const float* pred, const float* y,
                        int64_t y_stride, const float* stats, int loss_kind, const float* gout, float* dh, float* dz,
                        float* dw, float* db, float* workspace, int accumulate, hipStream_t stream);
int geossl_property_bwd_dyn(int64_t N, int F, const int32_t* mol_ptr, int64_t B, int readout, int head, const float* W1,
                            const float* W2, const float* m, const float* z, const float* pred, const float* y,
                            int64_t y_stride, const float* stats, int loss_kind, const float* gout, float* dh, float* dz,
                            float* dw, float* db, float* workspace, int accumulate, const int32_t* dyn_N,
                            hipStream_t stream);
int geossl_property_targets(const float* y, int64_t M, int T, int task_id, const int64_t* mol_off,
                            const int32_t* src_off, int64_t B, float* out, hipStream_t stream);

int geossl_pair_head_width_ok(int F);
int64_t geossl_pair_head_workspace_floats(int64_t B);
int geossl_pair_head_fwd(const float* h, int64_t N, int F, const int32_t* mol_ptr, int64_t B, int readout, const float* w,
                         const float* b, const float* y, float* m, float* z, float* workspace, float* loss,
                         hipStream_t stream);
int geossl_pair_head_predict(const float* h, int64_t N, int F, const int32_t* mol_ptr, int64_t B, int readout,
                             const float* w, const float* b, float* z, hipStream_t stream);
int geossl_pair_head_bwd(int64_t N, int F, const int32_t* mol_ptr, int64_t B, int readout, const float* w, const float* m,
                         const float* z, const float* y, const float* gout, float* dh, float* dw, float* db,
                         float* workspace, int accumulate, hipStream_t stream);
int geossl_pair_head_fwd_dyn(const float* h, int64_t N, int F, const int32_t* mol_ptr, int64_t B, int readout,
                             const float* w, const float* b, const float* y, float* m, float* z, float* workspace,
                             float* loss, const int32_t* dyn_N, hipStream_t stream);
int geossl_pair_head_predict_dyn(const float* h, int64_t N, int F, const int32_t* mol_ptr, int64_t B, int readout,
                                 const float* w, const float* b, float* z, const int32_t* dyn_N, hipStream_t stream);
int geossl_pair_head_bwd_dyn(int64_t N, int F, const int32_t* mol_ptr, int64_t B, int readout, const float* w,
                             const float* m, const float* z, const float* y, const float* gout, float* dh, float* dw,
                             float* db, float* workspace, int accumulate, const int32_t* dyn_N, hipStream_t stream);

int geossl_torsion_head_width_ok(int F);
int64_t geossl_torsion_head_fwd_workspace_floats(int64_t T);
int64_t geossl_torsion_head_bwd_workspace_floats(int64_t N, int F);
int geossl_torsion_head_fwd(const float* h, int64_t N, int F, const float* W, const float* bias, const int64_t* tri0,
                            const int64_t* tri1, const int64_t* tri2, const float* angle, int64_t T, float* proj,
                            float* pred, float* res, float* workspace, float* loss, hipStream_t stream);
int geossl_torsion_head_fwd_dyn(const float* h, int64_t N, int F, const float* W, const float* bias, const int64_t* tri0,
                                const int64_t* tri1, const int64_t* tri2, const float* angle, int64_t T, float* proj,
                                float* pred, float* res, float* workspace, float* loss, const int32_t* dyn_N,
                                const int32_t* dyn_T, hipStream_t stream);
int geossl_torsion_head_bwd(const float* h, int64_t N, int F, const float* W, const int64_t* tri0, const int64_t* tri1,
                            const int64_t* tri2, int64_t T, const float* res, const int32_t* mol_ptr, int64_t B,
                            const float* gout, float* dh, float* dW, float* db, float* workspace, int accumulate,
                            hipStream_t stream);
int geossl_torsion_head_bwd_dyn(const float* h, int64_t N, int F, const float* W, const int64_t* tri0,
                                const int64_t* tri1, const int64_t* tri2, int64_t T, const float* res,
                                const int32_t* mol_ptr, int64_t B, const float* gout, float* dh, float* dW, float* db,
                                float* workspace, int accumulate, const int32_t* dyn_N, const int32_t* dyn_T,
                                hipStream_t stream);
int geossl_triple_angles(const float* pos, int64_t N, const int64_t* tri0, const int64_t* tri1, const int64_t* tri2,
                         int64_t T, float* angle, hipStream_t stream);
int geossl_gather_triples(const int32_t* tri_src, int64_t stride, const float* angle_src, const int32_t* t_src_off,
                          const int32_t* t_ptr, const int32_t* mol_ptr, int64_t B, int64_t* tri0, int64_t* tri1,
                          int64_t* tri2, float* angle_dst, hipStream_t stream);

int geossl_sparse_pairs_build(const float* pos, const int32_t* mol_ptr, int64_t B, int64_t N, int max_n, float r2,
                              int cap, float cutoff, int64_t capacity, int32_t* mol_cnt, int32_t* up_cnt,
                              int32_t* lo_cnt, int32_t* pair_i, int32_t* pair_j, float* pair_d, float* pair_c,
                              uint8_t* pair_flag, int32_t* inc_ptr, int32_t* inc_pair, uint32_t* inc_src,
                              int32_t* n_pairs, hipStream_t stream);
int geossl_sparse_pairs_build_dyn(const float* pos, const int32_t* mol_ptr, int64_t B, int64_t N, int max_n, float r2,
                                  int cap, float cutoff, int64_t capacity, int32_t* mol_cnt, int32_t* up_cnt,
                                  int32_t* lo_cnt, int32_t* pair_i, int32_t* pair_j, float* pair_d, float* pair_c,
                                  uint8_t* pair_flag, int32_t* inc_ptr, int32_t* inc_pair, uint32_t* inc_src,
                                  int32_t* n_pairs, const int32_t* dyn_N, hipStream_t stream);

int geossl_pair_geometry_live(const float* pos, const int32_t* mol_ptr, const int32_t* pair_ptr, int64_t B, int max_n,
                              float r2, int cap, float cutoff, float* pair_d, float* pair_c, uint8_t* pair_flag,
                              int32_t* mol_live, hipStream_t stream);
int geossl_live_pairs_build(const float* pair_d, const float* pair_c, const uint8_t* pair_flag, const int32_t* pair_i,
                            const int32_t* pair_j, const int32_t* mol_ptr, const int32_t* pair_ptr,
                            const int32_t* mol_live, int64_t B, int64_t P, float cutoff, const int32_t* dyn_P,
                            float* live_d, float* live_c, uint8_t* live_flag, int32_t* live_i, int32_t* live_j,
                            int32_t* row_slot, int32_t* n_live, hipStream_t stream);
int geossl_cfconv_filter_fwd_rows(const float* pair_d, const float* pair_c, int64_t P, const GeosslFilterWeights* w, int L,
                                  int F, int G, const float* offset, float coeff, float* T, float* Wf,
                                  const int32_t* dyn_P, const int32_t* row_slot, hipStream_t stream);
int geossl_gather_live_rows(const float* src, const int32_t* row_slot, const int32_t* n_live, int64_t P, int L, int F,
                            float* dst, hipStream_t stream);

int geossl_cfconv_aggregate_sparse(const float* x, const float* Wf, const int32_t* inc_ptr, const int32_t* inc_pair,
                                   const uint32_t* inc_src, int64_t N, int F, int swap, float* out,
                                   hipStream_t stream);
int geossl_cfconv_aggregate_sparse_dyn(const float* x, const float* Wf, const int32_t* inc_ptr,
                                       const int32_t* inc_pair, const uint32_t* inc_src, int64_t N, int F, int swap,
                                       float* out, const int32_t* dyn_N, hipStream_t stream);
int geossl_pair_position_grad_sparse(const float* pos, const float* pair_d, const float* dd, const int32_t* inc_ptr,
                                     const int32_t* inc_pair, const uint32_t* inc_src, int64_t N, int64_t P, int L,
                                     float* dpos, hipStream_t stream);

#ifdef __cplusplus
}
#endif
#endif
```

Baseline: 426,400.

## Compute NCSN first-layer weight grads per atom instead of per super-edge

Adds a per-atom backward path for the DDM/NCSN loss head and makes it the default (the old row-fused path now needs GEOSSL_NCSN_ROW_BWD). The fused row kernel stops doing the per-edge dz1·[h_u,h_v] outer-product MMA and the dz1 LDS staging. It writes dfeat directly, and the in-layer scalar grads move into a pipelined 'narrow' step. An incidence gather then sums dfeat per atom into a workspace, and a separate k_ncsn_atoms kernel forms the o1_w gradient from per-atom dz and h. The aim is to shrink the weight-gradient GEMM from the number of super-edges to the number of atoms and to free LDS and registers in the main kernel. The cost is extra kernel launches and 2*N*F of workspace traffic.

```diff
diff --git a/geossl_amd/NCSN.py b/geossl_amd/NCSN.py
--- a/geossl_amd/NCSN.py
+++ b/geossl_amd/NCSN.py
@@ -64,6 +64,10 @@
         for ev, _keep in _SIDE["pending"]:
             torch.cuda.current_stream().wait_event(ev)
         _SIDE["pending"].clear()
+
+
+def _row_bwd():
+    return _env("GEOSSL_NCSN_ROW_BWD") is not None
 
 
 class _NcsnLoss(torch.autograd.Function):
@@ -123,7 +127,20 @@
         acc = 1 if direct else 0
         split = (_env("GEOSSL_NCSN_SPLIT_BWD") is not None or _env("GEOSSL_ARITH_24BIT") is not None
                  or max(S, N) * Fd * 4 >= 2 ** 32)
-        if not split:
+        dh = None
+        want_dh = ctx.needs_input_grad[0]
+        if want_dh:
+            slot = ctx.grad_slot
+            dh = slot.rows(N, Fd, torch.float32, dev) if slot is not None else None
+            if dh is None:
+                dh = torch.empty(N, Fd, dtype=torch.float32, device=dev)
+        if not split and not _row_bwd():
+            ws1 = torch.empty(int(lib.geossl_ddm_loss_bwd_atoms_workspace_floats(S, N, Fd)), dtype=torch.float32, device=dev)
+            call("geossl_ddm_loss_bwd_atoms", ptr(h), ptr(sel.sei0), ptr(sel.sei1), S, N, Fd, C.byref(w), C.byref(sv),
+                 ptr(sel.stats), ctx.out_scale, ptr(gout), ptr(sel.inc_ptr), ptr(sel.inc_idx), ptr(dfeat), ptr(demb),
+                 ptr(grow), ptr(dh) if want_dh else None, C.byref(g), ptr(ws1), acc, st)
+            want_dh = False
+        elif not split:
             ws1 = torch.empty(int(lib.geossl_ddm_loss_bwd_fused_workspace_floats(S, Fd)), dtype=torch.float32, device=dev)
             call("geossl_ddm_loss_bwd_fused", ptr(h), ptr(sel.sei0), ptr(sel.sei1), S, N, Fd, C.byref(w), C.byref(sv),
                  ptr(sel.stats), ctx.out_scale, ptr(gout), ptr(dfeat), ptr(demb), ptr(grow), C.byref(g), ptr(ws1), acc, st)
@@ -132,12 +149,7 @@
             dz1 = torch.empty(S, Fd, dtype=torch.float32, device=dev)
             call("geossl_ddm_loss_bwd_rows", C.byref(w), C.byref(sv), S, Fd, ptr(sel.stats), ctx.out_scale, ptr(gout),
                  ptr(dz1), ptr(dfeat), ptr(demb), ptr(grow), st)
-        dh = None
-        if ctx.needs_input_grad[0]:
-            slot = ctx.grad_slot
-            dh = slot.rows(N, Fd, torch.float32, dev) if slot is not None else None
-            if dh is None:
-                dh = torch.empty(N, Fd, dtype=torch.float32, device=dev)
+        if want_dh:
             call("geossl_incidence_gather", ptr(dfeat), ptr(sel.inc_ptr), ptr(sel.inc_idx), N, Fd, ptr(dh), 0, st)
         if split:
             nfl = lib.geossl_ddm_loss_bwd_workspace_floats(S, Fd)
@@ -230,8 +242,8 @@
         lib = _lib.load()
         heads = (_lib.NcsnHeadBwd * 2)()
         keep, dhs = [], []
-        nws = int(lib.geossl_ddm_loss_bwd_fused_workspace_floats(S, Fd))
         dyn = ctx.dyn
+        nws = int(lib.geossl_ddm_loss_bwd_atoms_workspace_floats(S, sel.N if dyn is not None else N, Fd))
         dh_all = torch.empty(N, Fd, dtype=torch.float32, device=dev) if dyn is not None else None
         for k in range(2):
             hd = heads[k]
@@ -254,7 +266,7 @@
                 ptr(hs[k]), ctx.out_scale, ptr(dfeat), ptr(demb), ptr(grow), ptr(ws1), ptr(dh))
             keep += [dfeat, demb, grow, ws1]
             dhs.append(dh)
-        call("geossl_ddm_loss_bwd_fused2_dyn", C.byref(heads), ptr(sel.sei0), ptr(sel.sei1), S, sel.N if dyn is not None else N,
+        call("geossl_ddm_loss_bwd_fused2_dyn" if _row_bwd() else "geossl_ddm_loss_bwd_atoms2_dyn", C.byref(heads), ptr(sel.sei0), ptr(sel.sei1), S, sel.N if dyn is not None else N,
              Fd, ptr(sel.stats), ptr(gout), ptr(sel.inc_ptr), ptr(sel.inc_idx), 1 if direct else 0,
              None if dyn is None else dyn.n_super, None if dyn is None else dyn.n_atoms, st)
         head = ((dh_all, None) if dyn is not None else (dhs[0], dhs[1])) + (None,) * 11
diff --git a/geossl_amd/_lib.py b/geossl_amd/_lib.py
--- a/geossl_amd/_lib.py
+++ b/geossl_amd/_lib.py
@@ -170,6 +170,11 @@
     "geossl_ddm_loss_bwd_fused": (i32, [vp, vp, vp, i64, i64, i32, P(NcsnWeights), P(NcsnSaved), vp, f32, vp, vp, vp, vp,
                                         P(NcsnGrads), vp, i32, vp]),
     "geossl_incidence_gather": (i32, [vp, vp, vp, i64, i32, vp, i32, vp]),
+    "geossl_ddm_loss_bwd_atoms_workspace_floats": (i64, [i64, i64, i32]),
+    "geossl_ddm_loss_bwd_atoms": (i32, [vp, vp, vp, i64, i64, i32, P(NcsnWeights), P(NcsnSaved), vp, f32, vp, vp, vp, vp,
+                                        vp, vp, vp, P(NcsnGrads), vp, i32, vp]),
+    "geossl_ddm_loss_bwd_atoms2": (i32, [vp, vp, vp, i64, i64, i32, vp, vp, vp, vp, i32, vp]),
+    "geossl_ddm_loss_bwd_atoms2_dyn": (i32, [vp, vp, vp, i64, i64, i32, vp, vp, vp, vp, i32, vp, vp, vp]),
     "geossl_painn_edge_geom": (i32, [vp, vp, vp, i64, f32, vp, vp, i32, vp, vp, vp, vp]),
     "geossl_silu_fwd": (i32, [vp, i64, vp, vp]),
     "geossl_silu_bwd": (i32, [vp, vp, i64, vp, vp]),
diff --git a/geossl_amd/csrc/ncsn_bwd.hip b/geossl_amd/csrc/ncsn_bwd.hip
--- a/geossl_amd/csrc/ncsn_bwd.hip
+++ b/geossl_amd/csrc/ncsn_bwd.hip
@@ -20,9 +20,10 @@
 #define NB_MARK(slot) do {} while (0)
 #endif
 
-template <int NW>
+template <int NW, bool PER_ATOM = false>
 struct NbLds {
   static constexpr int F = 32 * NW, H = F / 2, KHS = (H + 15) / 16, HMB = (H + 31) / 32, KS = F / 16;
+  static constexpr int RING = PER_ATOM ? 4 : 3, NDEP = PER_ATOM ? 2 : 1;
   u32x4* zb;
   u32x4* dz2T;
   u32x4* fT;
@@ -40,20 +41,20 @@
     zb = reinterpret_cast<u32x4*>(smem);
     dz2T = zb + 2 * KHS * 2 * 64;
     fT = dz2T + HMB * 2 * 2 * 64;
-    dz1r = fT + 2 * NW * 2 * 2 * 64;
-    abT = dz1r + KS * 2 * 64;
+    dz1r = fT + (PER_ATOM ? 0 : 2 * NW * 2 * 2 * 64);
+    abT = dz1r + (PER_ATOM ? 0 : KS * 2 * 64);
     scal = reinterpret_cast<int4*>(abT + NW * 2 * 2 * 64);
-    pdv = reinterpret_cast<float*>(scal + 3 * TR);
-    dep = pdv + 3 * TR;
-    wls = dep + NW * TR;
+    pdv = reinterpret_cast<float*>(scal + RING * TR);
+    dep = pdv + RING * TR;
+    wls = dep + NDEP * NW * TR;
     eg = reinterpret_cast<int*>(wls + F);
     ef = eg + 4;
     ea = ef + 2 * NW;
     ec = ea + NW;
   }
   static size_t bytes() {
-    return (size_t)(2 * KHS * 2 + HMB * 4 + 2 * NW * 4 + KS * 2 + NW * 4) * 1024 + 3 * TR * sizeof(int4) +
-           (size_t)(3 * TR + NW * TR + F) * sizeof(float) + (size_t)(4 + 4 * NW) * sizeof(int);
+    return (size_t)(2 * KHS * 2 + HMB * 4 + (PER_ATOM ? 0 : 2 * NW * 4 + KS * 2) + NW * 4) * 1024 + RING * TR * sizeof(int4) +
+           (size_t)(RING * TR + NDEP * NW * TR + F) * sizeof(float) + (size_t)(4 + 4 * NW) * sizeof(int);
   }
 };
 
@@ -100,10 +101,12 @@
 __device__ __forceinline__ float pow2(int e) { return __builtin_amdgcn_ldexpf(1.0f, e); }
 constexpr int E_NONE = -100000;
 
-template <int NW, bool ROLE_A>
+template <int NW, bool ROLE_A, bool PER_ATOM = false>
 __device__ __forceinline__ void ncsn_bwd_body(const NcsnFusedArgs& a, const int S, const float* __restrict__ a_h) {
-  using L_t = NbLds<NW>;
-  constexpr int F = L_t::F, H = L_t::H, KHS = L_t::KHS, HMB = L_t::HMB, KS = L_t::KS, NT = 128 * NW;
+  using L_t = NbLds<NW, PER_ATOM>;
+  constexpr int F = L_t::F, H = L_t::H, KHS = L_t::KHS, HMB = L_t::HMB, KS = L_t::KS, NT = 128 * NW, RING = L_t::RING;
+  constexpr bool NARROW = ROLE_A != PER_ATOM;
+  const int wave_n = PER_ATOM ? NW : 0;
   extern __shared__ __attribute__((aligned(16))) uint8_t smem_raw[];
   const L_t L(smem_raw);
   const int tid = threadIdx.x, lane = tid & 63, j = lane & 31, kh = lane >> 5;
@@ -115,10 +118,10 @@
   const float scale = a.out_scale * (a.gout != nullptr ? a.gout[0] : 1.0f) / (float)a.divisor[0];
   const uint32_t col = 32 * nb + j;
 
-  Frag2 wreg[ROLE_A ? KHS : KS];
-  f32x16 accw1[ROLE_A ? NW : 1];
+  Frag2 wreg[ROLE_A ? KHS : (PER_ATOM ? 1 : KS)];
+  f32x16 accw1[ROLE_A && !PER_ATOM ? NW : 1];
   f32x16 accw2[ROLE_A ? 1 : HMB];
-  int E1[ROLE_A ? NW : 1];
+  int E1[ROLE_A && !PER_ATOM ? NW : 1];
   int E2 = E_NONE;
   int ew = 0;
   float bsum = 0.0f, dsum = 0.0f;
@@ -133,9 +136,11 @@
     e3 = scale_exponent(wave_max(m3));
   }
   if constexpr (ROLE_A) {
-    iw1 = a.w.in_w1[col];
-    ib1 = a.w.in_b1[col];
-    iw2 = a.w.in_w2[col];
+    if constexpr (NARROW) {
+      iw1 = a.w.in_w1[col];
+      ib1 = a.w.in_b1[col];
+      iw2 = a.w.in_w2[col];
+    }
     float raw[KHS][8];
     float wm = 0.0f, csum = 0.0f;
 #pragma unroll
@@ -155,11 +160,13 @@
     csum += __shfl_xor(csum, 32, 64);
     const int ecw = max(mag_exponent(wave_max(csum)), -80);
     if (lane == 0) L.ec[nb] = ecw;
-#pragma unroll
-    for (int kb = 0; kb < NW; ++kb) {
-      E1[kb] = E_NONE;
-#pragma unroll
-      for (int r = 0; r < 16; ++r) accw1[kb][r] = 0.0f;
+    if constexpr (!PER_ATOM) {
+#pragma unroll
+      for (int kb = 0; kb < NW; ++kb) {
+        E1[kb] = E_NONE;
+#pragma unroll
+        for (int r = 0; r < 16; ++r) accw1[kb][r] = 0.0f;
+      }
     }
 #pragma unroll
     for (int s = 0; s < 2; ++s)
@@ -169,19 +176,26 @@
         ident[s][q] = (k0 == j ? 0x3C00u : 0u) | (k1 == j ? 0x3C000000u : 0u);
       }
   } else {
-    float raw[KS][8];
-    float wm = 0.0f;
-#pragma unroll
-    for (int ks = 0; ks < KS; ++ks)
-#pragma unroll
-      for (int e = 0; e < 8; ++e) {
-        raw[ks][e] = a.w.o1_w[(size_t)(16 * ks + kperm(e, kh)) * (F + 1) + col];
-        wm = fmaxf(wm, fabsf(raw[ks][e]));
-      }
-    ew = scale_exponent(wave_max(wm));
-    const float sw = pow2(14 - ew);
-#pragma unroll
-    for (int ks = 0; ks < KS; ++ks) wreg[ks] = split8h_scaled(raw[ks], sw);
+    if constexpr (NARROW) {
+      iw1 = a.w.in_w1[col];
+      ib1 = a.w.in_b1[col];
+      iw2 = a.w.in_w2[col];
+    }
+    if constexpr (!PER_ATOM) {
+      float raw[KS][8];
+      float wm = 0.0f;
+#pragma unroll
+      for (int ks = 0; ks < KS; ++ks)
+#pragma unroll
+        for (int e = 0; e < 8; ++e) {
+          raw[ks][e] = a.w.o1_w[(size_t)(16 * ks + kperm(e, kh)) * (F + 1) + col];
+          wm = fmaxf(wm, fabsf(raw[ks][e]));
+        }
+      ew = scale_exponent(wave_max(wm));
+      const float sw = pow2(14 - ew);
+#pragma unroll
+      for (int ks = 0; ks < KS; ++ks) wreg[ks] = split8h_scaled(raw[ks], sw);
+    }
 #pragma unroll
     for (int e = 0; e < 8; ++e) {
       const int m = 16 * nb + 8 * kh + e;
@@ -224,11 +238,11 @@
         const float gr = valid ? pin(sc_g) * scale : 0.0f;
         EG = max(EG, mag_exponent(wave_max(fabsf(gr))));
         if (lane < TR) {
-          L.scal[(tt % 3) * TR + lane] = make_int4(sc_u, sc_v, __float_as_int(gr), __float_as_int(sc_e));
-          L.pdv[(tt % 3) * TR + lane] = sc_p;
+          L.scal[(tt % RING) * TR + lane] = make_int4(sc_u, sc_v, __float_as_int(gr), __float_as_int(sc_e));
+          L.pdv[(tt % RING) * TR + lane] = sc_p;
           if (valid) a.grow[row] = gr;
         }
-        if (lane == 0) L.eg[tt % 3] = EG;
+        if (lane == 0) L.eg[tt % RING] = EG;
       }
     }
   };
@@ -253,8 +267,8 @@
   };
   float hu[16], hv[16];
   auto request_gather = [&](int tt, int k4) {
-    if constexpr (!ROLE_A) {
-      const int2* sc = reinterpret_cast<const int2*>(L.scal + (tt % 3) * TR);
+    if constexpr (!ROLE_A && !PER_ATOM) {
+      const int2* sc = reinterpret_cast<const int2*>(L.scal + (tt % RING) * TR);
 #pragma unroll
       for (int r = 0; r < 16; ++r) {
         const int2 uv = sc[2 * crow4(r, k4)];
@@ -266,8 +280,8 @@
   auto build_zb = [&](int tt) {
     if constexpr (!ROLE_A) {
       if (nb < KHS) {
-        const float gr = __int_as_float(L.scal[(tt % 3) * TR + j].z);
-        const float sz = pow2(14 - e3 - __builtin_amdgcn_readfirstlane(L.eg[tt % 3]));
+        const float gr = __int_as_float(L.scal[(tt % RING) * TR + j].z);
+        const float sz = pow2(14 - e3 - __builtin_amdgcn_readfirstlane(L.eg[tt % RING]));
         const float av[8] = {a2raw[0].x, a2raw[0].y, a2raw[0].z, a2raw[0].w, a2raw[1].x, a2raw[1].y, a2raw[1].z, a2raw[1].w};
         float v[8];
 #pragma unroll
@@ -285,7 +299,7 @@
   };
   int EF = -40;
   auto build_fT = [&](int tt) {
-    if constexpr (!ROLE_A) {
+    if constexpr (!ROLE_A && !PER_ATOM) {
       float v[16];
       float m = 0.0f;
 #pragma unroll
@@ -305,6 +319,31 @@
         u32x4* dst = L.fT + (size_t)((((tt & 1) * NW + nb) * 2 + s) * 2) * 64 + lane;
         dst[0] = f.h;
         dst[64] = f.l;
+      }
+    }
+  };
+
+  auto narrow = [&](int tt, int k4) {
+    if constexpr (PER_ATOM && !ROLE_A) {
+      const int4* sc = L.scal + (tt % RING) * TR;
+      const float* pdr = L.pdv + (tt % RING) * TR;
+      const float* dp_ = L.dep + (PER_ATOM ? (tt & 1) * TR * NW : 0);
+#pragma unroll
+      for (int i = 0; i < 16; ++i) {
+        const int rl = 4 * k4 + i;
+        float de = 0.0f;
+#pragma unroll
+        for (int n2 = 0; n2 < NW; ++n2) de += dp_[rl * NW + n2];
+        const float pd = pdr[rl];
+        const float pre = fmaf(iw1, pd, ib1);
+        s_w2 = fmaf(de, fmaxf(pre, 0.0f), s_w2);
+        const float dp = pre > 0.0f ? de * iw2 : 0.0f;
+        s_w1 = fmaf(dp, pd, s_w1);
+        s_b1 += dp;
+        if (wave == wave_n && j == i) {
+          s_g += __int_as_float(sc[rl].z);
+          s_d += de;
+        }
       }
     }
   };
@@ -337,7 +376,7 @@
     NB_MARK(0);
     lds_barrier();
     NB_MARK(1);
-    const int EGt = __builtin_amdgcn_readfirstlane(L.eg[t % 3]);
+    const int EGt = __builtin_amdgcn_readfirstlane(L.eg[t % RING]);
     if constexpr (ROLE_A) {
       put_scal(t + 2);
       const float kT = pow2(EGt + eC - 14);
@@ -363,7 +402,7 @@
       NB_MARK(5);
       float v[16];
       {
-        const int4* sc = L.scal + (t % 3) * TR;
+        const int4* sc = L.scal + (t % RING) * TR;
         float tb = 0.0f, td = 0.0f, am = 0.0f;
 #pragma unroll
         for (int r = 0; r < 16; ++r) {
@@ -413,16 +452,25 @@
           tp = mfma_f16(piece(da[1], pc), ident[1], tp);
 #pragma unroll
           for (int r = 0; r < 16; ++r) de = fmaf(tp[r], wl[r], de);
-#pragma unroll
-          for (int half = 0; half < 2; ++half)
-            L.dz1r[(size_t)((2 * nb + half) * 2 + pc) * 64 + lane] = pack8(tp, half);
+          if constexpr (!PER_ATOM) {
+#pragma unroll
+            for (int half = 0; half < 2; ++half)
+              L.dz1r[(size_t)((2 * nb + half) * 2 + pc) * 64 + lane] = pack8(tp, half);
+          }
         }
         de += __shfl_xor(de, 32, 64);
-        if (kh == 0) L.dep[j * NW + nb] = de * kT;
+        if (kh == 0) L.dep[(PER_ATOM ? (t & 1) * TR * NW : 0) + j * NW + nb] = de * kT;
       }
       NB_MARK(6);
-#pragma unroll
-      for (int kb = 0; kb < NW; ++kb) {
+      if constexpr (PER_ATOM) {
+#pragma unroll
+        for (int r = 0; r < 16; ++r) {
+          const int row = TR * t + crow4(r, k4);
+          if (row < S) a.dfeat[((uint32_t)row * (uint32_t)F + col)] = v[r] * kT;
+        }
+      }
+#pragma unroll
+      for (int kb = 0; kb < (PER_ATOM ? 0 : NW); ++kb) {
         const int En = EGt + __builtin_amdgcn_readfirstlane(L.ef[buf * NW + kb]);
         if (En != E1[kb]) {
           const float f = pow2(max(E1[kb] - En, -200));
@@ -462,6 +510,9 @@
       }
       NB_MARK(5);
       build_zb(t + 1);
+      if constexpr (PER_ATOM) {
+        if (t > t_begin) narrow(t - 1, k4);
+      }
       NB_MARK(6);
       build_fT(t + 1);
     }
@@ -472,9 +523,9 @@
     if constexpr (ROLE_A) {
       request_a1(t + 1, k4);
       load_scal(t + 3);
-      {
-        const int4* sc = L.scal + (t % 3) * TR;
-        const float* pdr = L.pdv + (t % 3) * TR;
+      if constexpr (!PER_ATOM) {
+        const int4* sc = L.scal + (t % RING) * TR;
+        const float* pdr = L.pdv + (t % RING) * TR;
 #pragma unroll
         for (int i = 0; i < 16; ++i) {
           const int rl = 4 * k4 + i;
@@ -500,7 +551,7 @@
       f32x16 acc0, acc1;
 #pragma unroll
       for (int r = 0; r < 16; ++r) acc0[r] = acc1[r] = 0.0f;
-      {
+      if constexpr (!PER_ATOM) {
         const u32x4* zs = L.dz1r + lane;
         Frag2 b0, bn;
         b0.h = zs[0]; b0.l = zs[64];
@@ -522,15 +573,17 @@
       for (int r = 0; r < 16; ++r) outp[r] = (acc0[r] + acc1[r]) * kD;
       const int row = TR * t + j;
       if (row < S) {
-        const uint32_t off = ((uint32_t)row * (uint32_t)F + 32 * nb + 4 * kh) * 4u;
-#pragma unroll
-        for (int q = 0; q < 4; ++q)
-          *reinterpret_cast<f32x4*>(reinterpret_cast<char*>(a.dfeat) + 32 * q + off) =
-              f32x4{outp[4 * q], outp[4 * q + 1], outp[4 * q + 2], outp[4 * q + 3]};
+        if constexpr (!PER_ATOM) {
+          const uint32_t off = ((uint32_t)row * (uint32_t)F + 32 * nb + 4 * kh) * 4u;
+#pragma unroll
+          for (int q = 0; q < 4; ++q)
+            *reinterpret_cast<f32x4*>(reinterpret_cast<char*>(a.dfeat) + 32 * q + off) =
+                f32x4{outp[4 * q], outp[4 * q + 1], outp[4 * q + 2], outp[4 * q + 3]};
+        }
         if (nb == 0 && kh == 0) {
           float de = 0.0f;
 #pragma unroll
-          for (int n2 = 0; n2 < NW; ++n2) de += L.dep[j * NW + n2];
+          for (int n2 = 0; n2 < NW; ++n2) de += L.dep[(PER_ATOM ? (t & 1) * TR * NW : 0) + j * NW + n2];
           a.demb[row] = de;
         }
       }
@@ -561,11 +614,14 @@
     }
     NB_MARK(4);
   }
+  if constexpr (PER_ATOM) {
+    if (t_begin < t_end) narrow(t_end - 1, opaque(4 * kh));
+  }
   const size_t pb = blockIdx.x;
   if constexpr (ROLE_A) {
     float* P1 = a.pw1 + pb * F * F;
 #pragma unroll
-    for (int kb = 0; kb < NW; ++kb) {
+    for (int kb = 0; kb < (PER_ATOM ? 0 : NW); ++kb) {
       const float f = pow2(max(E1[kb] + eC - 28, -200));
 #pragma unroll
       for (int r = 0; r < 16; ++r) P1[(size_t)(32 * nb + c_row(r, lane)) * F + 32 * kb + j] = accw1[kb][r] * f;
@@ -575,22 +631,41 @@
       a.pb1[pb * F + col] = sb;
       a.pd1[pb * F + col] = sd;
     }
-    float* Ps = a.psm + pb * (H + 3 * F + 2);
-    const float t_w2 = s_w2 + __shfl_xor(s_w2, 32, 64);
-    const float t_w1 = s_w1 + __shfl_xor(s_w1, 32, 64), t_b1 = s_b1 + __shfl_xor(s_b1, 32, 64);
-    if (kh == 0) {
-      Ps[H + col] = t_w2;
-      Ps[H + F + col] = t_w1;
-      Ps[H + 2 * F + col] = t_b1;
-    }
-    if (wave == 0) {
-      const float tg = wave_sum(s_g), td = wave_sum(s_d);
-      if (lane == 0) {
-        Ps[H + 3 * F] = tg;
-        Ps[H + 3 * F + 1] = td;
+    if constexpr (!PER_ATOM) {
+      float* Ps = a.psm + pb * (H + 3 * F + 2);
+      const float t_w2 = s_w2 + __shfl_xor(s_w2, 32, 64);
+      const float t_w1 = s_w1 + __shfl_xor(s_w1, 32, 64), t_b1 = s_b1 + __shfl_xor(s_b1, 32, 64);
+      if (kh == 0) {
+        Ps[H + col] = t_w2;
+        Ps[H + F + col] = t_w1;
+        Ps[H + 2 * F + col] = t_b1;
+      }
+      if (wave == wave_n) {
+        const float tg = wave_sum(s_g), td = wave_sum(s_d);
+        if (lane == 0) {
+          Ps[H + 3 * F] = tg;
+          Ps[H + 3 * F + 1] = td;
+        }
       }
     }
   } else {
+    if constexpr (PER_ATOM) {
+      float* Ps = a.psm + pb * (H + 3 * F + 2);
+      const float t_w2 = s_w2 + __shfl_xor(s_w2, 32, 64);
+      const float t_w1 = s_w1 + __shfl_xor(s_w1, 32, 64), t_b1 = s_b1 + __shfl_xor(s_b1, 32, 64);
+      if (kh == 0) {
+        Ps[H + col] = t_w2;
+        Ps[H + F + col] = t_w1;
+        Ps[H + 2 * F + col] = t_b1;
+      }
+      if (wave == wave_n) {
+        const float tg = wave_sum(s_g), td = wave_sum(s_d);
+        if (lane == 0) {
+          Ps[H + 3 * F] = tg;
+          Ps[H + 3 * F + 1] = td;
+        }
+      }
+    }
     float* P2 = a.pw2 + pb * H * F;
     const float f = pow2(max(E2 + e3 - 28, -200));
 #pragma unroll
@@ -631,6 +706,147 @@
   if (dyn_view != nullptr && blockIdx.y == 1) h += (size_t)(*dyn_view) * (32 * NW);
   if ((int)(threadIdx.x >> 6) < NW) ncsn_bwd_body<NW, true>(a, S, h);
   else ncsn_bwd_body<NW, false>(a, S, h);
+}
+
+template <int NW>
+__global__ __launch_bounds__(128 * NW) void k_ncsn_bwd_rows_atoms(NcsnFusedPair pr, const int32_t* __restrict__ dyn_S) {
+  const NcsnFusedArgs& a = pr.a[blockIdx.y];
+  const int S = dyn_count(a.S, dyn_S);
+  if ((int)(threadIdx.x >> 6) < NW) ncsn_bwd_body<NW, true, true>(a, S, nullptr);
+  else ncsn_bwd_body<NW, false, true>(a, S, nullptr);
+}
+
+struct NcsnAtomArgs {
+  const float* dz;
+  const float* h;
+  const float* w1;
+  float* dh;
+  float* pw1;
+};
+struct NcsnAtomPair { NcsnAtomArgs a[2]; };
+template <int NW>
+__global__ __launch_bounds__(128 * NW) void k_ncsn_atoms(NcsnAtomPair pr, int N, const int32_t* __restrict__ dyn_view) {
+  constexpr int F = 32 * NW, KS = F / 16;
+  __shared__ u32x4 dzr[KS][3][64];
+  __shared__ u32x4 hT[NW][2][3][64];
+  const NcsnAtomArgs& a = pr.a[blockIdx.y];
+  N = dyn_count(N, dyn_view);
+  const size_t voff = (dyn_view != nullptr && blockIdx.y == 1) ? (size_t)N * F : 0;
+  const float* __restrict__ Dz = a.dz + voff;
+  const float* __restrict__ H = a.h + voff;
+  float* __restrict__ dh = a.dh != nullptr ? a.dh + voff : nullptr;
+  const int lane = threadIdx.x & 63, j = lane & 31, kh = lane >> 5;
+  const int wave = __builtin_amdgcn_readfirstlane((int)(threadIdx.x >> 6));
+  const bool role_h = wave < NW;
+  const int w = role_h ? wave : wave - NW;
+  const int col = 32 * w + j;
+  const int ntiles = (N + 31) / 32;
+  const int per = (ntiles + (int)gridDim.x - 1) / (int)gridDim.x;
+  const int t_begin = (int)blockIdx.x * per, t_end = min(ntiles, t_begin + per);
+  if (role_h) {
+    Frag3 wreg[KS];
+#pragma unroll
+    for (int ks = 0; ks < KS; ++ks) {
+      float raw[8];
+#pragma unroll
+      for (int e = 0; e < 8; ++e) raw[e] = a.w1[(size_t)(16 * ks + kperm(e, kh)) * (F + 1) + col];
+      wreg[ks] = split8(raw);
+    }
+    f32x4 zrow[2][2];
+    auto request = [&](int t) {
+      const float* zr = Dz + (size_t)min(32 * t + j, N - 1) * F + 32 * w + 4 * kh;
+#pragma unroll
+      for (int s = 0; s < 2; ++s)
+#pragma unroll
+        for (int p = 0; p < 2; ++p) zrow[s][p] = *reinterpret_cast<const f32x4*>(zr + 16 * s + 8 * p);
+    };
+    if (t_begin < t_end) request(t_begin);
+    for (int t = t_begin; t < t_end; ++t) {
+      const int a0 = 32 * t;
+#pragma unroll
+      for (int s = 0; s < 2; ++s) {
+        const float v[8] = {zrow[s][0].x, zrow[s][0].y, zrow[s][0].z, zrow[s][0].w,
+                            zrow[s][1].x, zrow[s][1].y, zrow[s][1].z, zrow[s][1].w};
+        const Frag3 f = split8(v);
+        dzr[2 * w + s][0][lane] = f.h;
+        dzr[2 * w + s][1][lane] = f.m;
+        dzr[2 * w + s][2][lane] = f.l;
+      }
+      lds_barrier();
+      if (t + 1 < t_end) request(t + 1);
+      f32x16 acc0, acc1;
+#pragma unroll
+      for (int r = 0; r < 16; ++r) acc0[r] = acc1[r] = 0.0f;
+#pragma unroll
+      for (int ks = 0; ks < KS; ++ks) {
+        Frag3 b;
+        b.h = dzr[ks][0][lane]; b.m = dzr[ks][1][lane]; b.l = dzr[ks][2][lane];
+        mma6x2(acc0, acc1, wreg[ks], b);
+      }
+      if (dh != nullptr && a0 + j < N) {
+        float* dst = dh + (size_t)(a0 + j) * F + 32 * w + 4 * kh;
+#pragma unroll
+        for (int q = 0; q < 4; ++q)
+          *reinterpret_cast<f32x4*>(dst + 8 * q) = f32x4{acc0[4 * q] + acc1[4 * q], acc0[4 * q + 1] + acc1[4 * q + 1],
+                                                         acc0[4 * q + 2] + acc1[4 * q + 2], acc0[4 * q + 3] + acc1[4 * q + 3]};
+      }
+      lds_barrier();
+    }
+  } else {
+    f32x16 accw[NW];
+#pragma unroll
+    for (int kb = 0; kb < NW; ++kb)
+#pragma unroll
+      for (int r = 0; r < 16; ++r) accw[kb][r] = 0.0f;
+    float zcol[2][8], hcol[2][8];
+    auto request = [&](int t) {
+#pragma unroll
+      for (int s = 0; s < 2; ++s)
+#pragma unroll
+        for (int e = 0; e < 8; ++e) {
+          const size_t o = (size_t)min(32 * t + 16 * s + 8 * kh + e, N - 1) * F + col;
+          zcol[s][e] = Dz[o];
+          hcol[s][e] = H[o];
+        }
+    };
+    if (t_begin < t_end) request(t_begin);
+    for (int t = t_begin; t < t_end; ++t) {
+      const int a0 = 32 * t;
+      Frag3 zT[2];
+#pragma unroll
+      for (int s = 0; s < 2; ++s) {
+        float zc[8], hc[8];
+#pragma unroll
+        for (int e = 0; e < 8; ++e) {
+          const bool live = a0 + 16 * s + 8 * kh + e < N;
+          const float z = pin(zcol[s][e]), hv = pin(hcol[s][e]);
+          zc[e] = live ? z : 0.0f;
+          hc[e] = live ? hv : 0.0f;
+        }
+        zT[s] = split8(zc);
+        const Frag3 g = split8(hc);
+        hT[w][s][0][lane] = g.h;
+        hT[w][s][1][lane] = g.m;
+        hT[w][s][2][lane] = g.l;
+      }
+      lds_barrier();
+      if (t + 1 < t_end) request(t + 1);
+#pragma unroll
+      for (int s = 0; s < 2; ++s)
+#pragma unroll
+        for (int kb = 0; kb < NW; ++kb) {
+          Frag3 b;
+          b.h = hT[kb][s][0][lane]; b.m = hT[kb][s][1][lane]; b.l = hT[kb][s][2][lane];
+          mma6(accw[kb], zT[s], b);
+        }
+      lds_barrier();
+    }
+    float* P1 = a.pw1 + (size_t)blockIdx.x * F * F;
+#pragma unroll
+    for (int kb = 0; kb < NW; ++kb)
+#pragma unroll
+      for (int r = 0; r < 16; ++r) P1[(size_t)(32 * w + c_row(r, lane)) * F + 32 * kb + j] = accw[kb][r];
+  }
 }
 
 __device__ __forceinline__ void ncsn_reduce_all_block(const ReduceMulti& m, int nblk, int accumulate,
@@ -801,3 +1017,110 @@
                                     dyn_view);
   return 0;
 }
+
+static int64_t atoms_dz_offset(int64_t S, int F) { return (geossl_ddm_loss_bwd_fused_workspace_floats(S, F) + 63) / 64 * 64; }
+
+extern "C" int64_t geossl_ddm_loss_bwd_atoms_workspace_floats(int64_t S, int64_t N, int F) {
+  return atoms_dz_offset(S, F) + 2 * N * (int64_t)F;
+}
+
+namespace {
+int bwd_atoms(const GeosslNcsnHeadBwd* heads, int nh, const int64_t* sei0, const int64_t* sei1, int64_t S, int64_t N, int F,
+              const int64_t* stats_divisor, const float* gout, const int64_t* inc_ptr, const int32_t* inc_idx,
+              int accumulate, const int32_t* dyn_S, const int32_t* dyn_view, hipStream_t stream) {
+  if (S <= 0) return 0;
+  if (heads == nullptr || N <= 0 || (F != 32 && F != 64 && F != 128)) return (int)hipErrorInvalidValue;
+  if (S * (int64_t)F * 4 >= ((int64_t)1 << 32) || N * (int64_t)F * 4 >= ((int64_t)1 << 32)) return (int)hipErrorInvalidValue;
+  const int nb = nh == 2 ? (fused_blocks(S) + 1) / 2 : fused_blocks(S), H = F / 2;
+  const int64_t dz_off = atoms_dz_offset(S, F);
+  NcsnFusedPair pr;
+  NcsnAtomPair pa;
+  for (int k = 0; k < 2; ++k) {
+    const GeosslNcsnHeadBwd& hd = heads[k < nh ? k : 0];
+    if (hd.h == nullptr || hd.dfeat == nullptr || hd.workspace == nullptr) return (int)hipErrorInvalidValue;
+    NcsnFusedArgs& x = pr.a[k];
+    x.h = hd.h; x.sei0 = sei0; x.sei1 = sei1; x.S = (int)S; x.w = hd.w; x.sv = hd.saved; x.divisor = stats_divisor;
+    x.out_scale = hd.out_scale; x.gout = gout; x.dfeat = hd.dfeat; x.demb = hd.demb; x.grow = hd.grow;
+    x.pw1 = hd.workspace;
+    x.pd1 = x.pw1 + (size_t)nb * F * F;
+    x.pb1 = x.pd1 + (size_t)nb * F;
+    x.pw2 = x.pb1 + (size_t)nb * F;
+    x.pb2 = x.pw2 + (size_t)nb * H * F;
+    x.psm = x.pb2 + (size_t)nb * H;
+    NcsnAtomArgs& y = pa.a[k];
+    y.dz = hd.workspace + dz_off; y.h = hd.h; y.w1 = hd.w.o1_w; y.dh = hd.dh; y.pw1 = x.pw1;
+  }
+#define LAUNCH_ROWS(NWV)                                                                                              \
+  do {                                                                                                                \
+    allow_big_lds(&k_ncsn_bwd_rows_atoms<NWV>);                                                                       \
+    hipLaunchKernelGGL((k_ncsn_bwd_rows_atoms<NWV>), dim3(nb, nh), dim3(128 * NWV), (NbLds<NWV, true>::bytes()),      \
+                       stream, pr, dyn_S);                                                                            \
+  } while (0)
+  if (F == 128) LAUNCH_ROWS(4); else if (F == 64) LAUNCH_ROWS(2); else LAUNCH_ROWS(1);
+#undef LAUNCH_ROWS
+  GEOSSL_CHECK_LAUNCH();
+  float* dz0 = const_cast<float*>(pa.a[0].dz);
+  float* dz1 = const_cast<float*>(pa.a[1].dz);
+  const int rc = nh == 2 ? launch_incidence_gather2(heads[0].dfeat, heads[1].dfeat, inc_ptr, inc_idx, N, F, dz0, dz1,
+                                                    stream, dyn_view)
+                         : geossl_incidence_gather(heads[0].dfeat, inc_ptr, inc_idx, N, F, dz0, 0, stream);
+  if (rc) return rc;
+#define LAUNCH_ATOMS(NWV) \
+  hipLaunchKernelGGL((k_ncsn_atoms<NWV>), dim3(nb, nh), dim3(128 * NWV), 0, stream, pa, (int)N, dyn_view)
+  if (F == 128) LAUNCH_ATOMS(4); else if (F == 64) LAUNCH_ATOMS(2); else LAUNCH_ATOMS(1);
+#undef LAUNCH_ATOMS
+  GEOSSL_CHECK_LAUNCH();
+  ReduceMulti rm[2];
+  for (int k = 0; k < nh; ++k) {
+    const GeosslNcsnGrads* grads = &heads[k].grads;
+    const NcsnFusedArgs& x = pr.a[k];
+    float* o1w[1] = {grads->o1_w};
+    float* o1c[1] = {grads->o1_w + F};
+    float* o1b[1] = {grads->o1_b};
+    float* o2w[1] = {grads->o2_w};
+    float* o2b[1] = {grads->o2_b};
+    rm[k].add(x.pw1, F * F, F, F + 1, 1, o1w, 1);
+    rm[k].add(x.pd1, F, F, F, F + 1, o1c, 1);
+    rm[k].add(x.pb1, F, F, F, 1, o1b, 1);
+    rm[k].add(x.pw2, H * F, F, F, 1, o2w, 1);
+    rm[k].add(x.pb2, H, H, H, 1, o2b, 1);
+  }
+  const dim3 rgrid(rm[0].blocks() + (H + 3 * F + 2 + 3) / 4, nh);
+  if (nh == 2)
+    hipLaunchKernelGGL(k_ncsn_reduce_all2, rgrid, dim3(256), 0, stream, rm[0], rm[1], nb, accumulate, pr.a[0].psm,
+                       pr.a[1].psm, F, heads[0].grads, heads[1].grads);
+  else
+    hipLaunchKernelGGL(k_ncsn_reduce_all, rgrid, dim3(256), 0, stream, rm[0], nb, accumulate, pr.a[0].psm, F,
+                       heads[0].grads);
+  GEOSSL_CHECK_LAUNCH();
+  return 0;
+}
+}
+
+extern "C" int geossl_ddm_loss_bwd_atoms(const float* h, const int64_t* sei0, const int64_t* sei1, int64_t S, int64_t N,
+                                         int F, const GeosslNcsnWeights* w, const GeosslNcsnSaved* saved,
+                                         const int64_t* stats_divisor, float out_scale, const float* gout,
+                                         const int64_t* inc_ptr, const int32_t* inc_idx, float* dz1, float* demb,
+                                         float* grow, float* dh, const GeosslNcsnGrads* grads, float* workspace,
+                                         int accumulate, hipStream_t stream) {
+  if (w == nullptr || saved == nullptr || grads == nullptr) return (int)hipErrorInvalidValue;
+  GeosslNcsnHeadBwd hd;
+  hd.h = h; hd.w = *w; hd.saved = *saved; hd.out_scale = out_scale; hd.pad_ = 0.0f; hd.dfeat = dz1; hd.demb = demb;
+  hd.grow = grow; hd.grads = *grads; hd.workspace = workspace; hd.dh = dh;
+  return bwd_atoms(&hd, 1, sei0, sei1, S, N, F, stats_divisor, gout, inc_ptr, inc_idx, accumulate, nullptr, nullptr, stream);
+}
+
+extern "C" int geossl_ddm_loss_bwd_atoms2(const GeosslNcsnHeadBwd* heads, const int64_t* sei0, const int64_t* sei1,
+                                          int64_t S, int64_t N, int F, const int64_t* stats_divisor, const float* gout,
+                                          const int64_t* inc_ptr, const int32_t* inc_idx, int accumulate,
+                                          hipStream_t stream) {
+  return bwd_atoms(heads, 2, sei0, sei1, S, N, F, stats_divisor, gout, inc_ptr, inc_idx, accumulate, nullptr, nullptr, stream);
+}
+
+extern "C" int geossl_ddm_loss_bwd_atoms2_dyn(const GeosslNcsnHeadBwd* heads, const int64_t* sei0, const int64_t* sei1,
+                                              int64_t S, int64_t N, int F, const int64_t* stats_divisor,
+                                              const float* gout, const int64_t* inc_ptr, const int32_t* inc_idx,
+                                              int accumulate, const int32_t* dyn_S, const int32_t* dyn_view,
+                                              hipStream_t stream) {
+  return bwd_atoms(heads, 2, sei0, sei1, S, N, F, stats_divisor, gout, inc_ptr, inc_idx, accumulate, dyn_S, dyn_view, stream);
+}
diff --git a/include/geossl_hip.h b/include/geossl_hip.h
--- a/include/geossl_hip.h
+++ b/include/geossl_hip.h
@@ -277,6 +277,19 @@
                               const GeosslNcsnGrads* grads, float* workspace, int accumulate, hipStream_t stream);
 int geossl_incidence_gather(const float* dfeat, const int64_t* inc_ptr, const int32_t* inc_idx, int64_t N, int F,
                             float* dh, int accumulate, hipStream_t stream);
+int64_t geossl_ddm_loss_bwd_atoms_workspace_floats(int64_t S, int64_t N, int F);
+int geossl_ddm_loss_bwd_atoms(const float* h, const int64_t* sei0, const int64_t* sei1, int64_t S, int64_t N, int F,
+                              const GeosslNcsnWeights* w, const GeosslNcsnSaved* saved, const int64_t* stats_divisor,
+                              float out_scale, const float* gout, const int64_t* inc_ptr, const int32_t* inc_idx,
+                              float* dz1, float* demb, float* grow, float* dh, const GeosslNcsnGrads* grads,
+                              float* workspace, int accumulate, hipStream_t stream);
+int geossl_ddm_loss_bwd_atoms2(const GeosslNcsnHeadBwd* heads, const int64_t* sei0, const int64_t* sei1, int64_t S,
+                               int64_t N, int F, const int64_t* stats_divisor, const float* gout, const int64_t* inc_ptr,
+                               const int32_t* inc_idx, int accumulate, hipStream_t stream);
+int geossl_ddm_loss_bwd_atoms2_dyn(const GeosslNcsnHeadBwd* heads, const int64_t* sei0, const int64_t* sei1, int64_t S,
+                                   int64_t N, int F, const int64_t* stats_divisor, const float* gout,
+                                   const int64_t* inc_ptr, const int32_t* inc_idx, int accumulate, const int32_t* dyn_S,
+                                   const int32_t* dyn_view, hipStream_t stream);
 
 int geossl_painn_edge_geom(const float* pos, const int64_t* idx_i, const int64_t* idx_j, int64_t E, float cutoff,
                            const float* offsets, const float* widths, int R, float* dir, float* fcut, float* phi,
```

After: 403,100. -5.5%, worse.
